# SuperbTUM/real-time-ReID-tracking

Hardware: AMD Instinct MI355X
Metric: crops/sec embedded + NxM distmat ms, ResNet18-SE 128x256 (higher is better)
Workload: dtype f16x3; 1 GPU; BASELINE configs[1]: ResNet18-SE embed 4096 distinct uint8 crops (128x256) per GPU + 4096x4096 L2 distmat; crops_per_gpu=4096, embed_dim=512, chunk=1024

## Files before the change

### include/reid_hip_debug.h

```cpp
#pragma once
#include "reid_hip.h"

#ifdef __cplusplus
extern "C" {
#endif

int reid_debug_set_switch(reid_ctx* ctx, const char* name, long long value);
int reid_debug_get_switch(reid_ctx* ctx, const char* name, long long* value);
int reid_debug_conv_f16(reid_ctx* ctx, int n, int h, int w, int cin, int cout, int r, int stride, int pad, int cfg, int iters,
                        float* ms_per_launch);
int reid_debug_conv_split(reid_ctx* ctx, int n, int h, int w, int c, int cout, int ablate, int iters, float* ms_per_launch);
int reid_debug_conv_f32(reid_ctx* ctx, int n, int h, int w, int cin, int cout, int r, int stride, int pad, int flags,
                        int variant, int iters, float* ms_per_launch);
int reid_debug_conv_c64(reid_ctx* ctx, int n, const float* x, const float* w_krsc, const float* scale, const float* shift,
                        const float* residual, int relu, float* out, float* stats);
int reid_debug_gemm_f16(reid_ctx* ctx, int m, int n, int k, int cfg, int iters, float* ms_per_launch,
                        unsigned long long* diag_host);
int reid_debug_linear(reid_ctx* ctx, int m, int n, int k, int mode, int iters, float* ms_per_launch);
int reid_debug_linear_rows(reid_ctx* ctx, const float* x, const float* w, const float* bias, const float* res, int m, int n, int k,
                           int mode, int flags, float* out);
int reid_debug_conv_layer(reid_ctx* ctx, const float* x, int n, int h, int w, int cin, const float* wgt, int cout, int r, int stride,
                          int pad, const float* scale, const float* shift, const float* residual, int relu, int relu_from, int pack_from,
                          int want_stats, const float* a_scale, const float* a_shift, int a_relu, float* out, uint16_t* packed,
                          float* stats, int* packed_written);
int reid_debug_norm_finish(reid_ctx* ctx, int form, int n, int hw, int c, int half, int tiles, const void* x, const float* stats,
                           const float* in_gamma, const float* in_beta, const float* bn_scale, const float* bn_shift, float* out,
                           uint16_t* out16, float* a_scale, float* a_shift);
int reid_debug_se_tail(reid_ctx* ctx, int form, int n, int hw, int c, int mid, int tiles, const float* stats, const float* w1,
                       const float* w2t, const void* y, const void* shortcut, float* out, uint16_t* out16, float* gate);
int reid_debug_sibling_tail(reid_ctx* ctx, int arch, int n, int h, int w, int c, const float* prm, const float* y, const float* shortcut,
                            float* out);
int reid_debug_gem_neck(reid_ctx* ctx, int f16, int n, int hw, int c, float p, const void* x, const float* scale, const float* shift,
                        float* gem_out, float* emb);
int reid_debug_stem(reid_ctx* ctx, int form, int is_u8, const void* x, int n, const float* w, const float* scale, const float* shift,
                    float* out, uint16_t* out16);
int reid_debug_resize_norm(reid_ctx* ctx, const uint8_t* packed, const long long* offsets, const int* hw, int n, int pitch, float* out);
int reid_debug_swin_crop_front(reid_ctx* ctx, const uint8_t* packed, const long long* offsets, const int* hw, int n, int pitch, int out_h,
                               int out_w, const float* mean_std6, const float* c1_w, const float* c1_b, float* out);
int reid_debug_swin_conv1(reid_ctx* ctx, const float* x, int n, int h, int w, const float* c1_w, const float* c1_b, float* out);
int reid_debug_maxpool(reid_ctx* ctx, int f16, const void* x, int n, int h, int w, int c, void* out);
int reid_debug_window_attn_cos(reid_ctx* ctx, int mode, const float* qkv, int n, int h, int w, int heads, int shifted, const float* bias,
                               const float* scale, float* out, uint16_t* out16);
int reid_debug_post_norm(reid_ctx* ctx, int side, const float* x, const float* y, int t, int c, const float* g, const float* b, int in_place,
                         float* out, uint16_t* out16);
int reid_debug_window_attn(reid_ctx* ctx, int form, const float* qkv, int n, int h, int w, int heads, int shifted, const float* pos169,
                           float* out, uint16_t* out16);
int reid_debug_layernorm(reid_ctx* ctx, int form, const float* x, int t, int c, const float* g, const float* b, float* out, uint16_t* out16);
int reid_debug_ln_linear(reid_ctx* ctx, const float* x, const float* ln_g, const float* ln_b, const float* w, const float* bias, int t, int c,
                         int n, float* out);
int reid_debug_swin_sfe(reid_ctx* ctx, const float* c1, int n, int h1, int w1, const float* in_g, const float* in_b, const float* bn_s,
                        const float* bn_t, const float* c2_w, const float* c2_b, const float* fc_w, const float* fc_b, float* ab, float* tok);
int reid_debug_swin_tail(reid_ctx* ctx, const float* x, int n, int ntok, const float* g, const float* b, float p, const float* bn_s,
                         const float* bn_t, float* gem, float* emb);
int reid_debug_swin_merge(reid_ctx* ctx, int stage, const float* x, int n, int h, int w, float* out);
int reid_debug_swin_fuse(reid_ctx* ctx, const float* sfe, const float* x1, const float* x2, const float* x3, const float* x4, int n, int h1,
                         int w1, void* a0, void* f3, void* f2, float* f1);
int reid_debug_two_linear_ablate(reid_ctx* ctx, int bits);
int reid_debug_two_linear(reid_ctx* ctx, const float* x, const float* w1, const float* b1, const float* w2, const float* b2,
                          const float* res, int m, int c, int hid, int act, int iters, float* out, float* ms, const float* ln_g,
                          const float* ln_b);
int reid_debug_select_exp(reid_ctx* ctx, int mode);
int reid_debug_knn_wide(reid_ctx* ctx, int enable, int force);
int reid_debug_conv_diag(reid_ctx* ctx, int enable, unsigned long long* out_host);
int reid_debug_mfma_shape(reid_ctx* ctx, int shape, int iters, int blocks, float* tflops);
int reid_debug_mfma_bare(reid_ctx* ctx, int shape, int zero, int iters, float* tflops);
int reid_debug_feed(reid_ctx* ctx, int mode, size_t footprint, int rowb, size_t stride, int iters, int inflight,
                    float* gbs_per_cu, float* tbs_chip);
int reid_debug_knn_merge(reid_ctx* ctx, const float* Dall, const int32_t* Iall, int world, int nq, int kk, int k, float* D,
                         int32_t* I);
int reid_debug_comm_loopback(reid_ctx** ctxs, int world);
int reid_debug_coissue(reid_ctx* ctx, int mode, int iters, int roles, double* cyc_mfma_wave, double* cyc_other_wave);

#ifdef __cplusplus
}
#endif
```

### real-time-reid-tracking_amd/_ffi.py

```python
import ctypes as C
import os

_HERE = os.path.dirname(os.path.abspath(__file__))
LIB_PATH = os.path.join(_HERE, "libreid_hip.so")
LIB_PATH = os.environ.get("REID_HIP_LIB", LIB_PATH)

METRIC_L2, METRIC_L2SQR, METRIC_COS_HALF, METRIC_COS, METRIC_DOT = range(5)
COMM_ID_BYTES = 128
K_CONV_GEMM, K_DIST_GEMM, K_ELEMENTWISE, K_SELECT = range(4)

_vp, _i, _sz = C.c_void_p, C.c_int, C.c_size_t
_SIGS = {
    "reid_last_error": (C.c_char_p, []),
    "reid_device_count": (_i, [C.POINTER(_i)]),
    "reid_ctx_create": (_i, [_i, C.POINTER(_vp)]),
    "reid_ctx_destroy": (_i, [_vp]),
    "reid_ctx_set_stream": (_i, [_vp, _vp]),
    "reid_ctx_set_null_stream": (_i, [_vp]),
    "reid_ctx_sync": (_i, [_vp]),
    "reid_device_sync": (_i, [_vp]),
    "reid_ctx_clear_fault": (_i, [_vp]),
    "reid_ctx_set_chunk": (_i, [_vp, _i]),
    "reid_ctx_set_precision": (_i, [_vp, _i]),
    "reid_ctx_precision_ok": (_i, [_vp, _i, _i]),
    "reid_ctx_fault_peek": (_i, [_vp, C.POINTER(_i)]),
    "reid_ctx_set_side_index": (_i, [_vp, _vp, _i]),
    "reid_malloc": (_i, [_vp, _sz, C.POINTER(_vp)]),
    "reid_free": (_i, [_vp, _vp]),
    "reid_memcpy_h2d": (_i, [_vp, _vp, _vp, _sz]),
    "reid_memcpy_d2h": (_i, [_vp, _vp, _vp, _sz]),
    "reid_timer_start": (_i, [_vp]),
    "reid_timer_stop": (_i, [_vp, C.POINTER(C.c_float)]),
    "reid_profile_enable": (_i, [_vp, _i]),
    "reid_profile_reset": (_i, [_vp]),
    "reid_profile_get": (_i, [_vp, _i, C.POINTER(C.c_double), C.POINTER(C.c_longlong), C.POINTER(C.c_double),
                              C.POINTER(C.c_double)]),
    "reid_seres18_load": (_i, [_vp, _vp, _sz, C.c_char_p]),
    "reid_seres18_dims": (_i, [_vp, C.POINTER(_i), C.POINTER(_i)]),
    "reid_embed_u8": (_i, [_vp, _vp, _i, _vp, _vp]),
    "reid_embed_u8_dev": (_i, [_vp, _vp, _i, _vp, _vp]),
    "reid_embed_ragged_u8": (_i, [_vp, _vp, _vp, _vp, _i, _vp, _vp]),
    "reid_embed_frame_u8": (_i, [_vp, _vp, _i, _i, _vp, _i, _vp, _vp]),
    "reid_embed_f32_nchw": (_i, [_vp, _vp, _i, _vp, _vp]),
    "reid_embed_f32_nchw_dev": (_i, [_vp, _vp, _i, _vp, _vp]),
    "reid_swin_load": (_i, [_vp, _vp, _sz, C.c_char_p]),
    "reid_swin_dims": (_i, [_vp, C.POINTER(_i), C.POINTER(_i)]),
    "reid_swin_embed_f32_nchw": (_i, [_vp, _vp, _i, _i, _i, _vp, _vp]),
    "reid_swin_embed_f32_nchw_dev": (_i, [_vp, _vp, _i, _i, _i, _vp, _vp]),
    "reid_swin_embed_ragged_u8": (_i, [_vp, _vp, _vp, _vp, _i, _i, _i, _vp, _vp, _vp]),
    "reid_swin_embed_frame_u8": (_i, [_vp, _vp, _i, _i, _vp, _i, _i, _i, _vp, _vp, _vp]),
    "reid_ctx_set_debug_keep": (_i, [_vp, _i]),
    "reid_debug_stage": (_i, [_vp, _i, _vp, _sz, C.POINTER(_sz)]),
    "reid_debug_swin_stage": (_i, [_vp, _i, _vp, _sz, C.POINTER(_sz)]),
    "reid_distmat": (_i, [_vp, _vp, _i, _vp, _i, _i, _i, _vp]),
    "reid_distmat_dev": (_i, [_vp, _vp, _i, _vp, _i, _i, _i, _vp]),
    "reid_argmin_rows": (_i, [_vp, _vp, _i, _vp, _i, _i, _i, _vp, _vp]),
    "reid_argmin_rows_dev": (_i, [_vp, _vp, _i, _vp, _i, _i, _i, _vp, _vp]),
    "reid_knn": (_i, [_vp, _vp, _i, _vp, _i, _i, _i, _vp, _vp]),
    "reid_knn_dev": (_i, [_vp, _vp, _i, _vp, _i, _i, _i, _vp, _vp]),
    "reid_descriptor_f32_nchw": (_i, [_vp, _vp, _i, _i, _vp]),
    "reid_descriptor_f32_nchw_dev": (_i, [_vp, _vp, _i, _i, _vp]),
    "reid_cam_debias": (_i, [_vp, _vp, _vp, _i, _i, C.c_float, _i]),
    "reid_cam_debias_dev": (_i, [_vp, _vp, _vp, _i, _i, C.c_float, _i]),
    "reid_smooth_tracklets": (_i, [_vp, _vp, _vp, _vp, _i, _i, C.c_float]),
    "reid_smooth_tracklets_dev": (_i, [_vp, _vp, _vp, _vp, _i, _i, C.c_float]),
    "reid_bank_create": (_i, [_vp, _i, _i, _i, C.POINTER(_vp)]),
    "reid_bank_destroy": (_i, [_vp]),
    "reid_bank_update": (_i, [_vp, _vp, _vp, _vp, _i]),
    "reid_bank_update_dev": (_i, [_vp, _vp, _vp, _vp, _i]),
    "reid_bank_clear": (_i, [_vp, _vp, _vp, _i]),
    "reid_bank_count": (_i, [_vp, _i, C.POINTER(_i)]),
    "reid_bank_cost": (_i, [_vp, _vp, _vp, _i, _vp, _i, _i, C.c_float, _vp]),
    "reid_bank_cost_dev": (_i, [_vp, _vp, _vp, _i, _vp, _i, _i, C.c_float, _vp]),
    "reid_host_alloc": (_i, [_vp, _sz, C.POINTER(_vp)]),
    "reid_host_free": (_i, [_vp, _vp]),
    "reid_frame_submit": (_i, [_vp, _i, _vp, _vp, _vp, _i]),
    "reid_frame_cost": (_i, [_vp, _i, _vp, _vp, _i, _i, C.c_float, _vp, _vp, _i]),
    "reid_frame_cost_groups": (_i, [_vp, _i, _i, _vp, _vp, _vp, _vp, _i, C.c_float, _vp, _vp, _i]),
    "reid_frame_match_stream": (_i, [_vp, _i]),
    "reid_frame_fetch": (_i, [_vp, _i, _vp, _vp, _vp]),
    "reid_frame_gather": (_i, [_vp, _i, _i]),
    "reid_frame_update": (_i, [_vp, _i, _vp, _vp, _vp, _i]),
    "reid_rerank_jaccard": (_i, [_vp, _vp, _i, _i, _i, _i, _vp, _vp]),
    "reid_rerank_jaccard_dev": (_i, [_vp, _vp, _i, _i, _i, _i, _vp, _vp]),
    "reid_diou": (_i, [_vp, _vp, _vp, _i, _vp]),
    "reid_diou_cost": (_i, [_vp, _vp, _i, _vp, _i, _vp]),
    "reid_rank_eval": (_i, [_vp, _vp, _vp, _vp, _i, _vp, _vp, _vp, _i, _i, _vp, _vp, _vp]),
    "reid_rank_eval_dev": (_i, [_vp, _vp, _vp, _vp, _i, _vp, _vp, _vp, _i, _i, _vp, _vp, _vp]),
    "reid_comm_unique_id": (_i, [_vp]),
    "reid_comm_init": (_i, [_vp, _i, _i, _vp]),
    "reid_comm_info": (_i, [_vp, C.POINTER(_i), C.POINTER(_i)]),
    "reid_comm_destroy": (_i, [_vp]),
    "reid_allgather_dev": (_i, [_vp, _vp, _vp, _sz]),
    "reid_allgather_rows_dev": (_i, [_vp, _vp, _i, _sz, _vp, _vp, C.POINTER(_i)]),
    "reid_allreduce_f64": (_i, [_vp, C.POINTER(C.c_double), _i, _i]),
    "reid_knn_gallery_sharded_dev": (_i, [_vp, _vp, _i, _vp, _i, _i, _i, _i, _vp, _vp]),
    "reid_conv2d_nhwc": (_i, [_vp, _vp, _i, _i, _i, _i, _vp, _i, _i, _i, _i, _i, _vp, _vp, _vp, _i, _vp]),
    "reid_gemm_nt": (_i, [_vp, _vp, _i, _vp, _i, _i, _vp, _vp]),
}
EXPORTS = tuple(sorted(_SIGS))

DEBUG_LIB_PATH = os.path.join(_HERE, "libreid_hip_debug.so")
DEBUG_EXPORTS = ("reid_debug_coissue", "reid_debug_comm_loopback", "reid_debug_conv_c64", "reid_debug_conv_layer", "reid_debug_conv_split", "reid_debug_conv_diag", "reid_debug_conv_f16", "reid_debug_conv_f32",
                 "reid_debug_feed", "reid_debug_gem_neck", "reid_debug_gemm_f16", "reid_debug_knn_merge", "reid_debug_knn_wide", "reid_debug_layernorm", "reid_debug_linear", "reid_debug_linear_rows", "reid_debug_ln_linear", "reid_debug_maxpool", "reid_debug_mfma_bare", "reid_debug_mfma_shape", "reid_debug_norm_finish", "reid_debug_post_norm", "reid_debug_resize_norm", "reid_debug_se_tail", "reid_debug_stem", "reid_debug_sibling_tail", "reid_debug_swin_conv1", "reid_debug_swin_crop_front", "reid_debug_swin_fuse", "reid_debug_swin_merge", "reid_debug_swin_sfe", "reid_debug_swin_tail", "reid_debug_select_exp", "reid_debug_set_switch", "reid_debug_get_switch", "reid_debug_two_linear", "reid_debug_two_linear_ablate", "reid_debug_window_attn", "reid_debug_window_attn_cos")

_lib = None
_dbg = None


class ReidHipError(RuntimeError):
    status = None


def lib():
    global _lib
    if _lib is None:
        if not os.path.exists(LIB_PATH):
            raise ReidHipError(
                "HIP extension missing: %s (build it with `python -c 'import __graft_entry__ as g; g.build()'` "
                "or `make -C real-time-reid-tracking_amd/csrc`); there is no CPU fallback" % LIB_PATH)
        l = C.CDLL(LIB_PATH, mode=C.RTLD_GLOBAL)
        for name, (res, args) in _SIGS.items():
            fn = getattr(l, name)
            fn.restype = res
            fn.argtypes = args
        _lib = l
    return _lib


def debug_lib():
    global _dbg
    if _dbg is None:
        lib()
        if not os.path.exists(DEBUG_LIB_PATH):
            raise ReidHipError("debug library missing: %s (make -C real-time-reid-tracking_amd/csrc)" % DEBUG_LIB_PATH)
        _dbg = C.CDLL(DEBUG_LIB_PATH)
    return _dbg


def check(status):
    if status != 0:
        msg = lib().reid_last_error()
        err = ReidHipError("libreid_hip status %d: %s" % (status, msg.decode() if msg else "?"))
        err.status = int(status)
        raise err
```

### real-time-reid-tracking_amd/csrc/api.hip

```cpp
#include "reid_internal.h"
#include "siblings_f16.h"
#include <dlfcn.h>
#include <mutex>
#include <stdarg.h>
#include <stdio.h>
#include <string.h>
#include <stdlib.h>
#include <sstream>

static thread_local char g_err[1024] = "";

void reid_set_error(const char* fmt, ...) {
    va_list ap;
    va_start(ap, fmt);
    vsnprintf(g_err, sizeof(g_err), fmt, ap);
    va_end(ap);
}

extern "C" const char* reid_last_error(void) { return g_err; }

extern "C" int reid_device_count(int* n) {
    ARG_CHECK(n);
    HIP_TRY(hipGetDeviceCount(n));
    return REID_OK;
// ... 636 lines not shown
    return launch_gemm_f32(ctx, amode, E_CONV, p, REID_K_CONV_GEMM, flops, bytes);
}

int conv_weights_fresh(reid_ctx* ctx, const float* d_w) {
    auto it = ctx->split_w.find(d_w);
    if (it != ctx->split_w.end()) {
        HIP_TRY(hipStreamSynchronize(ctx->stream));
        (void)hipFree(it->second);
        ctx->split_w.erase(it);
    }
    return REID_OK;
}

int conv_weights_splittable(reid_ctx* ctx, const float* h_w, size_t count, const char* who) {
    if (ctx->precision != 2) return REID_OK;
    for (size_t i = 0; i < count; ++i)
        if (!(fabsf(h_w[i]) * 2048.0f < 65504.0f)) {
            reid_set_error("%s: weight %zu (%g) is outside the range the fp32-class arithmetic (reid_ctx_set_precision 2) can split "
                           "(|w| 2^11 < 65504); use mode 0", who, i, (double)h_w[i]);
            return REID_ERR_ARG;
        }
    return REID_OK;
}

static int split_weights_of(reid_ctx* ctx, const float* wgt, int Cout, int taps, int Cin, const _Float16** out) {
    auto it = ctx->split_w.find(wgt);
    if (it == ctx->split_w.end()) {
        void* w16;
        HIP_TRY(hipMalloc(&w16, (size_t)Cout * taps * ctx->split_terms * Cin * 2));
        REID_TRY(launch_split_weights(ctx, wgt, Cout, taps, Cin, ctx->split_terms, (_Float16*)w16));
        it = ctx->split_w.emplace(wgt, w16).first;
    }
    *out = (const _Float16*)it->second;
    return REID_OK;
}

#ifdef REID_EXPERIMENTS
static int seres18_chain_layer4(reid_ctx* ctx, int n, const Se18Block& ka, const Se18Block& kb, const _Float16* in16, const float* sc,
                                float* y, float* out_a, float* out, float* stats) {
    const int H = 16, W = 8, hw = 128, C = 512, SK = 4, nnt = C / 128;
    const int nmt = (n * hw + 255) / 256;
    _Float16 *c1_16, *a16;
    float* skws;
    int* cnt;
    REID_TRY(ctx_ws(ctx, "split.c1", (size_t)n * hw * C * 2 * 2, (void**)&c1_16));
    REID_TRY(ctx_ws(ctx, "chain.a16", (size_t)n * hw * C * 2 * 2, (void**)&a16));
    const size_t part = (size_t)nmt * nnt * SK * 256 * 128;
    REID_TRY(ctx_ws(ctx, "chain.splitk", 4 * part * sizeof(float), (void**)&skws));
    const bool fresh = ctx->ws.find("chain.cnt") == ctx->ws.end();
    REID_TRY(ctx_ws(ctx, "chain.cnt", (4 * 1024 + 64 + 8 * 64) * sizeof(int), (void**)&cnt));
    if (fresh) HIP_TRY(hipMemsetAsync(cnt, 0, (4 * 1024 + 64 + 8 * 64) * sizeof(int), ctx->stream));
    ChainParams cp;
    memset(&cp, 0, sizeof(cp));
    cp.n_img = n;
    cp.flags = ctx->chain;
    cp.counters = cnt + 4 * 1024;
    cp.fault = ctx->fault;
    auto conv = [&](int idx, const _Float16* a, int cin, const float* wgt, const float* scale, const float* shift, const float* res, int relu,
                    float* stats_out, _Float16* pack) -> int {
        Gemm16Params& q = cp.conv[idx];
        q.H = H; q.W = W; q.Cin = 3 * cin; q.R = 3; q.S = 3; q.stride = 1; q.pad = 1; q.Ho = H; q.Wo = W;
        q.M = n * hw; q.N = C; q.K = 9 * 3 * cin; q.ldb = q.K;
        q.split_terms = 3;
        q.A = a;
        REID_TRY(split_weights_of(ctx, wgt, C, 9, cin, &q.B));
        q.C32 = y; q.ldc = C;
        q.col_scale = scale; q.col_shift = shift; q.res32 = res; q.relu = relu; q.relu_from = 0;
        q.stats = stats_out;
        q.acc_scale = 1.0f / 2048.0f;
        q.zero_page = ctx->se18.zero_page;
        q.pack16 = pack; q.pack_from = 0;
        q.split_k = SK; q.splitk_ws = skws + (size_t)idx * part; q.splitk_cnt = cnt + idx * 1024;
        q.fault = ctx->fault;
        return REID_OK;
    };
    REID_TRY(conv(0, in16, ka.cin, ka.conv1_w, ka.bn1_scale, ka.bn1_shift, nullptr, 1, nullptr, c1_16));
    REID_TRY(conv(1, c1_16, C, ka.conv2_w, ka.bn2_scale, ka.bn2_shift, nullptr, 0, stats, nullptr));
    REID_TRY(conv(2, a16, C, kb.conv1_w, kb.bn1_scale, kb.bn1_shift, nullptr, 1, nullptr, c1_16));
    REID_TRY(conv(3, c1_16, C, kb.conv2_w, kb.bn2_scale, kb.bn2_shift, out_a, 1, stats, nullptr));
    const int slices = 2;
    auto se = [&](int idx, const Se18Block& k, const float* shortcut, float* o, _Float16* pk) {
        ChainElem& e = cp.el[idx];
        e.x = y; e.stats = stats; e.sc = shortcut; e.g = k.se_w1; e.b = k.se_w2; e.out = o; e.packed = pk;
        e.c = C; e.half = 0; e.hw = hw; e.tiles = 1; e.mid = k.mid; e.slices = slices;
    };
    se(0, ka, sc, out_a, a16);
    se(1, kb, out_a, out, nullptr);
    const int conv_items = nmt * nnt * SK, se_items = n * slices;
    const int kinds[6] = {0, 0, 2, 0, 0, 2}, idxs[6] = {0, 1, 0, 2, 3, 1};
    const int targets[6] = {0, nnt * SK, nnt * SK, slices, nnt * SK, nnt * SK};
    int first = 0;
    for (int s = 0; s < 6; ++s) {
        ChainStage& st = cp.st[s];
        st.kind = kinds[s]; st.idx = idxs[s]; st.first = first; st.items = kinds[s] == 0 ? conv_items : se_items;
        st.dep = s - 1; st.target = targets[s]; st.sk = SK;
        first += st.items;
    }
    cp.n_stages = 6;
    cp.total_items = first;
    prof_begin(ctx, REID_K_CONV_GEMM, 2.0 * n * hw * C * 9.0 * (ka.cin + 3.0 * C), 0.0);
    const int st = launch_chain(ctx, cp, W);
    prof_end(ctx);
    return st;
}
#endif

struct Se18Bufs {
    float *stem, *pool, *t[4], *stats, *a_scale, *a_shift, *se, *gem;
    float* stage[11];
};

static int seres18_forward(reid_ctx* ctx, const void* x, bool is_u8, int n, float* d_emb, float* d_logits) {
    Se18Weights& w = ctx->se18;
    if (!w.loaded) {
        reid_set_error("reid_embed_*: call reid_seres18_load first");
        return REID_ERR_STATE;
    }
    Se18Bufs b;
    const size_t per = 131072;
    const bool keep = ctx->debug_keep != 0;
    REID_TRY(ctx_ws(ctx, "se18.stem", (size_t)n * 524288 * 4, (void**)&b.stem));
    REID_TRY(ctx_ws(ctx, "se18.pool", (size_t)n * per * 4, (void**)&b.pool));
    const int nt = keep ? 1 : 4;
    float* tbase = nullptr;
    REID_TRY(ctx_ws(ctx, "se18.t", (size_t)n * per * 4 * (keep ? 4 * 8 : 4), (void**)&tbase));
    REID_TRY(ctx_ws(ctx, "se18.stats", (size_t)n * 2048 * 4, (void**)&b.stats));
    REID_TRY(ctx_ws(ctx, "se18.ascale", (size_t)n * 512 * 4, (void**)&b.a_scale));
    REID_TRY(ctx_ws(ctx, "se18.ashift", (size_t)n * 512 * 4, (void**)&b.a_shift));
    REID_TRY(ctx_ws(ctx, "se18.se", (size_t)n * 512 * 4, (void**)&b.se));
    REID_TRY(ctx_ws(ctx, "se18.gem", (size_t)n * 512 * 4, (void**)&b.gem));
    (void)nt;

    const bool pool_fused = ctx->f32_conv == 1 && ctx->f32_stem_pool && ctx->debug_keep != 1;
    _Float16* cur16 = nullptr;
    const bool split_mode = ctx->precision == 2 && w.arch == 0 && ctx->f32_conv == 1;
    if (split_mode) REID_TRY(ctx_ws(ctx, "split.cur", (size_t)n * per * 2 * 2, (void**)&cur16));
    const bool stem_split = split_mode && pool_fused && ctx->stem_split;
    if (stem_split) {
        REID_TRY(launch_stem_split(ctx, x, is_u8, n, w.stem_w, w.stem_scale, w.stem_shift, b.pool, cur16));
    } else if (pool_fused) {
        REID_TRY(launch_stem_f32(ctx, x, is_u8, n, w.stem_w, w.stem_scale, w.stem_shift, b.pool, true));
    } else if (ctx->f32_conv == 1) {
        REID_TRY(launch_stem_f32(ctx, x, is_u8, n, w.stem_w, w.stem_scale, w.stem_shift, b.stem, false));
    } else {
        REID_TRY(conv_gemm(ctx, is_u8 ? A_STEM_U8 : A_STEM_F32, x, n, IMG_H, IMG_W, 3, w.stem_w, 64, 7, 7, 2, 3, 192, nullptr,
                           nullptr, 0, w.stem_scale, w.stem_shift, nullptr, 0, nullptr, b.stem));
    }
    if (!pool_fused) REID_TRY(launch_maxpool3s2(ctx, b.stem, n, 128, 64, 64, b.pool));
    b.stage[0] = b.stem;
    b.stage[1] = b.pool;

    const float* cur = b.pool;
    int H = 64, W = 32;
    if (split_mode && !stem_split) REID_TRY(launch_split_pack(ctx, b.pool, (long long)n * 64 * 32, 64, cur16));
    for (int i = 0; i < 8; ++i) {
        const Se18Block& k = w.blk[i];
#ifdef REID_EXPERIMENTS
        if (i == 6 && (ctx->chain & 1) && cur16 && !keep && n <= 64 && ctx->pack_epilogue && ctx->split_terms == 3) {
            float* fr[3];
            int nf = 0;
            for (int j = 0; j < 4 && nf < 3; ++j)
                if (tbase + (size_t)j * n * per != cur) fr[nf++] = tbase + (size_t)j * n * per;
            float *sc = fr[0], *y = fr[1], *out_a = fr[2], *out = const_cast<float*>(cur);
            REID_TRY(conv_gemm(ctx, A_IM2COL, cur, n, H, W, k.cin, k.ds_w, k.c, 1, 1, k.stride, 0, k.cin, nullptr, nullptr, 0, k.ds_scale, k.ds_shift,
                               nullptr, 0, nullptr, sc, 0, cur16));
            REID_TRY(seres18_chain_layer4(ctx, n, k, w.blk[7], cur16, sc, y, out_a, out, b.stats));
            b.stage[8] = out_a;
            b.stage[9] = out;
            cur = out;
            break;
        }
#endif
        float* tb[4];
        for (int j = 0; j < 4; ++j) tb[j] = tbase + ((size_t)(keep ? i * 4 : 0) + j) * n * per;
        float* free_[3];
        int nf = 0;
        for (int j = 0; j < 4 && nf < 3; ++j)
            if (tb[j] != cur) free_[nf++] = tb[j];
        float* c1 = free_[0];
        float* y = free_[1];
        float* sc = free_[2];
        const int Ho = (H + 2 - 3) / k.stride + 1, Wo = (W + 2 - 3) / k.stride + 1;
        const int hw = Ho * Wo, tiles = hw / 128;
        const int half = k.ibn ? k.c / 2 : 0;
        _Float16* c1_16 = nullptr;
        if (ctx->f32_conv == 1) {
            bool packed_c1 = false;
            if (cur16 && !keep && ctx->pack_epilogue) REID_TRY(ctx_ws(ctx, "split.c1", (size_t)n * hw * k.c * 2 * 2, (void**)&c1_16));
            if (k.ibn) {
                REID_TRY(conv_gemm(ctx, A_IM2COL, cur, n, H, W, k.cin, k.conv1_w, k.c, 3, 3, k.stride, 1, 9 * k.cin, nullptr, nullptr,
                                   0, w.ep + (size_t)i * 1024, w.ep + (size_t)i * 1024 + 512, nullptr, 1, b.stats, c1, half, cur16,
                                   c1_16, half, &packed_c1));
                if (cur16 && !keep) {
                    if (!c1_16) REID_TRY(ctx_ws(ctx, "split.c1", (size_t)n * hw * k.c * 2 * 2, (void**)&c1_16));
                    REID_TRY(launch_in_apply_pack(ctx, c1, b.stats, n, tiles, k.c, half, hw, k.in_gamma, k.in_beta, c1_16, packed_c1));
                } else {
                    REID_TRY(launch_in_apply(ctx, c1, b.stats, n, tiles, k.c, half, hw, k.in_gamma, k.in_beta));
                }
            } else {
                REID_TRY(conv_gemm(ctx, A_IM2COL, cur, n, H, W, k.cin, k.conv1_w, k.c, 3, 3, k.stride, 1, 9 * k.cin, nullptr, nullptr,
                                   0, k.bn1_scale, k.bn1_shift, nullptr, 1, nullptr, c1, 0, cur16, c1_16, 0, &packed_c1));
                if (!packed_c1) c1_16 = nullptr;
            }
            REID_TRY(conv_gemm(ctx, A_IM2COL, c1, n, Ho, Wo, k.c, k.conv2_w, k.c, 3, 3, 1, 1, 9 * k.c, nullptr, nullptr, 0,
                               k.bn2_scale, k.bn2_shift, k.ds ? nullptr : cur, k.ds ? 0 : 1, b.stats, y, 0, c1_16));
        } else {
        REID_TRY(conv_gemm(ctx, A_IM2COL, cur, n, H, W, k.cin, k.conv1_w, k.c, 3, 3, k.stride, 1, 9 * k.cin, nullptr, nullptr, 0,
                           nullptr, nullptr, nullptr, 0, b.stats, c1));
        REID_TRY(launch_norm_finalize(ctx, b.stats, n, tiles, k.c, half, hw, k.in_gamma, k.in_beta, k.bn1_scale, k.bn1_shift,
                                      b.a_scale, b.a_shift));
        REID_TRY(conv_gemm(ctx, A_IM2COL, c1, n, Ho, Wo, k.c, k.conv2_w, k.c, 3, 3, 1, 1, 9 * k.c, b.a_scale, b.a_shift, 1,
                           k.bn2_scale, k.bn2_shift, k.ds ? nullptr : cur, k.ds ? 0 : 1, b.stats, y));
        }
        const float* shortcut = cur;
        if (k.ds) {
            REID_TRY(conv_gemm(ctx, A_IM2COL, cur, n, H, W, k.cin, k.ds_w, k.c, 1, 1, k.stride, 0, k.cin, nullptr, nullptr, 0,
                               k.ds_scale, k.ds_shift, nullptr, 0, nullptr, sc, 0, cur16));
            shortcut = sc;
        }
        float* out = c1;
        if (w.arch == 1) {
            REID_TRY(launch_ta_tail(ctx, y, shortcut, n, Ho, Wo, k.c, k.ta, out));
        } else if (w.arch == 2) {
            REID_TRY(launch_ema_tail(ctx, y, shortcut, n, Ho, Wo, k.c, k.ema, out));
        } else if (ctx->f32_conv == 1) {
            bool fp32_read = true;
            if (cur16 && !keep && i < 7 && w.blk[i + 1].ds && ctx->pack_epilogue) {
                const Se18Block& nx = w.blk[i + 1];
                fp32_read = !(conv_split_path(ctx, n, Ho, Wo, nx.cin, nx.c, 3, 3, nx.stride, 1) &&
                              conv_split_path(ctx, n, Ho, Wo, nx.cin, nx.c, 1, 1, nx.stride, 0));
            }
            REID_TRY(launch_se_tail(ctx, b.stats, n, tiles, k.c, k.mid, hw, k.se_w1, k.se_w2, y, shortcut, fp32_read ? out : nullptr,
                                    i < 7 ? cur16 : nullptr));
        } else {
            REID_TRY(launch_se_finalize(ctx, b.stats, n, tiles, k.c, k.mid, hw, k.se_w1, k.se_w2, b.se));
            REID_TRY(launch_se_combine(ctx, y, shortcut, b.se, n, hw, k.c, out));
        }
        b.stage[2 + i] = out;
        cur = out;
        H = Ho;
        W = Wo;
    }
    REID_TRY(launch_gem_neck(ctx, cur, n, H * W, 512, w.gem_p, w.neck_scale, w.neck_shift, b.gem, d_emb));
    {
        const int32_t* d_cam;
        REID_TRY(ctx_take_side(ctx, n, w.num_cams, "reid_embed (camera bias)", &d_cam));
        if (d_cam) REID_TRY(launch_add_indexed_rows(ctx, d_emb, n, 1, 512, w.cam_bias, d_cam, w.cam_factor));
    }
    b.stage[10] = b.gem;
    if (d_logits) {
        if (!w.cls_w) {
            reid_set_error("logits requested but the weight blob has no classifier (cls.w)");
            return REID_ERR_STATE;
        }
        GemmParams p;
        memset(&p, 0, sizeof(p));
        p.A = d_emb; p.lda = 512;
        p.B = w.cls_w; p.ldb = 512;
        p.M = n; p.N = w.num_class; p.K = 512;
        p.C = d_logits; p.ldc = w.num_class;
        REID_TRY(launch_gemm_f32(ctx, A_DENSE, E_BIAS, p, REID_K_CONV_GEMM, 2.0 * n * w.num_class * 512,
                                 ((double)n * 512 + (double)w.num_class * 512 + (double)n * w.num_class) * 4.0));
    }
    ctx->last_n = n;
    ctx->last_f16 = false;
    for (int s = 0; s < 11; ++s) ctx->stage_ptr[s] = b.stage[s];
    return REID_OK;
}

struct SiblingsF16Api {
    decltype(&siblings_f16_ta_workspace_bytes) ta_bytes = nullptr;
    decltype(&siblings_f16_ta_tail) ta = nullptr;
    decltype(&siblings_f16_ema_tail) ema = nullptr;
};
static int siblings_f16_api(const SiblingsF16Api** out) {
    static std::mutex m;
    static SiblingsF16Api api;
    std::lock_guard<std::mutex> lk(m);
    if (!api.ta) {
        Dl_info info;
        std::string path = "libreid_hip_siblings_f16.so";
        if (dladdr((const void*)&siblings_f16_api, &info) && info.dli_fname) {
            const std::string self = info.dli_fname;
            const size_t slash = self.rfind('/');
            if (slash != std::string::npos) path = self.substr(0, slash + 1) + path;
        }
        void* h = dlopen(path.c_str(), RTLD_NOW | RTLD_LOCAL);
        if (!h) {
            reid_set_error("CARes18-IBN / EMARes18-IBN in the fp16-storage mode need %s beside libreid_hip.so: %s", path.c_str(), dlerror());
            return REID_ERR_STATE;
        }
        auto b = (decltype(api.ta_bytes))dlsym(h, "siblings_f16_ta_workspace_bytes");
        auto t = (decltype(api.ta))dlsym(h, "siblings_f16_ta_tail");
        auto e = (decltype(api.ema))dlsym(h, "siblings_f16_ema_tail");
        if (!b || !t || !e) {
            dlclose(h);
            reid_set_error("%s lacks siblings_f16_ta_workspace_bytes / siblings_f16_ta_tail / siblings_f16_ema_tail", path.c_str());
            return REID_ERR_STATE;
        }
        api.ta_bytes = b;
        api.ema = e;
        api.ta = t;
    }
    *out = &api;
    return REID_OK;
}

static int launch_sibling_tail_f16(reid_ctx* ctx, const SiblingsF16Api* api, int arch, const _Float16* y, const _Float16* sc, int n, int H,
                                   int W, int C, const float* prm, _Float16* out) {
    ARG_CHECK(api && y && sc && prm && out && out != y && out != sc);
    void* ws = nullptr;
    if (arch == 1) {
        const size_t bytes = api->ta_bytes(n, H, W, C);
        ARG_CHECK(bytes > 0);
        REID_TRY(ctx_ws(ctx, "ta16.ws", bytes, &ws));
    }
    prof_begin(ctx, REID_K_ELEMENTWISE, 0, (double)n * H * W * C * 2.0 * 4.0);
    const hipError_t e = arch == 1 ? api->ta(ctx->stream, y, sc, n, H, W, C, prm, ws, out) : api->ema(ctx->stream, y, sc, n, H, W, C, prm, out);
    prof_end(ctx);
    HIP_TRY(e);
    return REID_OK;
}

int conv_gemm16(reid_ctx* ctx, int amode, const _Float16* x, int n, int H, int W, int Cin, const _Float16* wgt, int Cout,
                       int R, int S, int stride, int pad, int K, const float* col_scale, const float* col_shift,
                       const _Float16* residual, int relu, float* stats, _Float16* out, int Hp, int Wp) {
    Gemm16Params p;
    memset(&p, 0, sizeof(p));
    p.A = x;
    p.H = H; p.W = W; p.Cin = Cin; p.R = R; p.S = S; p.stride = stride; p.pad = pad; p.Hp = Hp; p.Wp = Wp;
    p.Ho = (H + 2 * pad - R) / stride + 1;
    p.Wo = (W + 2 * pad - S) / stride + 1;
    p.B = wgt; p.ldb = amode == A16_STEM ? 256 : K;
    p.M = n * p.Ho * p.Wo; p.N = Cout; p.K = K;
    p.C = out; p.ldc = Cout;
    p.col_scale = col_scale; p.col_shift = col_shift; p.residual = residual; p.relu = relu; p.stats = stats;
    p.zero_page = ctx->se18.zero_page;
    p.diag = ctx->conv_diag;
    const double ktrue = (double)R * S * (amode == A16_STEM ? 3 : Cin);
    const double flops = 2.0 * p.M * Cout * ktrue;
    const double bytes = ((double)n * H * W * (amode == A16_STEM ? 4 : Cin) + (double)p.M * Cout + (double)Cout * ktrue +
                          (residual ? (double)p.M * Cout : 0.0)) * 2.0;
    if (amode == A16_IM2COL && ctx->f16_halo && conv3x3_f16_supported(p)) {
        if (ctx->f16_halo == 2 || Cout >= 128) return launch_conv3x3_f16(ctx, p, REID_K_CONV_GEMM, flops, bytes);
    }
    return launch_gemm_f16(ctx, amode, p, REID_K_CONV_GEMM, flops, bytes);
}

static const int PAD_H = 262, PAD_W = 136;

static int seres18_forward_f16(reid_ctx* ctx, const void* x, bool is_u8, int n, float* d_emb, float* d_logits) {
    Se18Weights& w = ctx->se18;
    if (!w.loaded) {
        reid_set_error("reid_embed_*: call reid_seres18_load first");
        return REID_ERR_STATE;
    }
    typedef _Float16 f16;
    const size_t per = 131072;
    const bool keep = ctx->debug_keep != 0;
    const bool sibling = w.arch != 0;
    const SiblingsF16Api* sib = nullptr;
    if (sibling) REID_TRY(siblings_f16_api(&sib));
    f16 *pad_in, *stem, *pool, *tbase;
    float *stats, *a_scale, *a_shift, *se, *gem;
    REID_TRY(ctx_ws(ctx, "se18h.pad", (size_t)n * PAD_H * PAD_W * 4 * 2, (void**)&pad_in));
    REID_TRY(ctx_ws(ctx, "se18h.stem", (size_t)n * 524288 * 2, (void**)&stem));
    REID_TRY(ctx_ws(ctx, "se18h.pool", (size_t)n * per * 2, (void**)&pool));
    REID_TRY(ctx_ws(ctx, "se18h.t", (size_t)n * per * 2 * (keep ? 4 * 8 : 4), (void**)&tbase));
    REID_TRY(ctx_ws(ctx, "se18.stats", (size_t)n * 2048 * 4, (void**)&stats));
    REID_TRY(ctx_ws(ctx, "se18.ascale", (size_t)n * 512 * 4, (void**)&a_scale));
    REID_TRY(ctx_ws(ctx, "se18.ashift", (size_t)n * 512 * 4, (void**)&a_shift));
    REID_TRY(ctx_ws(ctx, "se18.se", (size_t)n * 512 * 4, (void**)&se));
    REID_TRY(ctx_ws(ctx, "se18.gem", (size_t)n * 512 * 4, (void**)&gem));

    const bool per_image_ok = n >= 128 || ctx->debug_keep == 2;
    const bool fused = ctx->f16_stem_fused && ctx->debug_keep != 1 && per_image_ok;
    if (is_u8 && fused && ctx->f16_stem_fused == 2) {
        REID_TRY(launch_stem_pool_f16(ctx, nullptr, (const uint8_t*)x, n, w.stem_w16s, w.stem_shift, pool));
    } else if (fused) {
        if (is_u8) REID_TRY(launch_prep_u8_pad_f16(ctx, (const uint8_t*)x, n, IMG_H, IMG_W, PAD_H, PAD_W, pad_in));
        else REID_TRY(launch_prep_f32_pad_f16(ctx, (const float*)x, n, IMG_H, IMG_W, PAD_H, PAD_W, pad_in));
        REID_TRY(launch_stem_pool_f16(ctx, pad_in, nullptr, n, w.stem_w16s, w.stem_shift, pool));
    } else {
        if (is_u8) REID_TRY(launch_prep_u8_pad_f16(ctx, (const uint8_t*)x, n, IMG_H, IMG_W, PAD_H, PAD_W, pad_in));
        else REID_TRY(launch_prep_f32_pad_f16(ctx, (const float*)x, n, IMG_H, IMG_W, PAD_H, PAD_W, pad_in));
        REID_TRY(conv_gemm16(ctx, A16_STEM, pad_in, n, IMG_H, IMG_W, 4, w.stem_w16, 64, 7, 7, 2, 3, 224, w.stem_scale,
                             w.stem_shift, nullptr, 0, nullptr, stem, PAD_H, PAD_W));
        REID_TRY(launch_maxpool3s2_f16(ctx, stem, n, 128, 64, 64, pool));
    }
    float* stage[11];
    stage[0] = (float*)stem;
    stage[1] = (float*)pool;

    const f16* cur = pool;
    int H = 64, W = 32;
    for (int i = 0; i < 8; ++i) {
// ... 735 lines not shown
```

### real-time-reid-tracking_amd/csrc/debug.hip

```cpp
#include "reid_internal.h"
#include <string.h>
#include <stdlib.h>
#include <vector>

namespace {
struct Switch { const char* name; int reid_ctx::* field; };
const Switch kSwitches[] = {
    {"f16_cfg", &reid_ctx::f16_cfg}, {"f16_lin_256", &reid_ctx::f16_lin_256}, {"f16_split_k", &reid_ctx::f16_split_k},
    {"bank_fast", &reid_ctx::bank_fast}, {"side_copy", &reid_ctx::side_copy}, {"f32_stem_pool", &reid_ctx::f32_stem_pool},
    {"stem_split", &reid_ctx::stem_split}, {"split_pair", &reid_ctx::split_pair}, {"split_lean_epi", &reid_ctx::split_lean_epi},
    {"knn_wide", &reid_ctx::knn_wide}, {"f16_loader_prio", &reid_ctx::f16_loader_prio}, {"f16_frag_ahead", &reid_ctx::f16_frag_ahead},
    {"pack_epilogue", &reid_ctx::pack_epilogue}, {"f16_wide_splitk", &reid_ctx::f16_wide_splitk}, {"f32_split_k", &reid_ctx::f32_split_k},
    {"swin_fold", &reid_ctx::swin_fold}, {"swin_stop", &reid_ctx::swin_stop}, {"select_two_pass", &reid_ctx::select_two_pass},
    {"split_terms", &reid_ctx::split_terms}, {"f32_conv", &reid_ctx::f32_conv}, {"swin_attn_mfma", &reid_ctx::swin_attn_mfma},
    {"swin_attn_split", &reid_ctx::swin_attn_split}, {"swin_two_linear", &reid_ctx::swin_two_linear},
    {"f16_loader_waves", &reid_ctx::f16_loader_waves}, {"f16_halo", &reid_ctx::f16_halo}, {"f16_stem_fused", &reid_ctx::f16_stem_fused},
    {"f16_se_tail", &reid_ctx::f16_se_tail}, {"f16_c64", &reid_ctx::f16_c64}, {"swin_chunk_cap", &reid_ctx::swin_chunk_cap},
    {"split_x3", &reid_ctx::split_x3}, {"x3_ablate", &reid_ctx::x3_ablate}, {"x3_unroll", &reid_ctx::x3_unroll}, {"x3_narrow", &reid_ctx::x3_narrow}, {"conv_x3s", &reid_ctx::conv_x3s}, {"x3s_sk_cap", &reid_ctx::x3s_sk_cap}, {"x3_l4_narrow_nmt", &reid_ctx::x3_l4_narrow_nmt}, {"split_x3_small", &reid_ctx::split_x3_small}, {"split_x3_min_blocks", &reid_ctx::split_x3_min_blocks}, {"f32_dist_bk16", &reid_ctx::f32_dist_bk16}, {"lin_x3", &reid_ctx::lin_x3},
    {"host_pipeline", &reid_ctx::host_pipeline}, {"x3_sk_cap", &reid_ctx::x3_sk_cap}, {"chain", &reid_ctx::chain}, {"split_gemm_min_tiles", &reid_ctx::split_gemm_min_tiles},
    {"rerank_hbm_acc", &reid_ctx::rerank_hbm_acc},
};
}

extern "C" int reid_debug_set_switch(reid_ctx* ctx, const char* name, long long value) {
    ARG_CHECK(ctx && name);
    CTX_GUARD(ctx);
    HIP_TRY(hipStreamSynchronize(ctx->stream));
    if (!strcmp(name, "knn_wide_min")) {
        ctx->knn_wide_min = value;
        return REID_OK;
    }
    for (const Switch& s : kSwitches)
        if (!strcmp(name, s.name)) {
            if (!strcmp(name, "split_terms") && value != 3 && value != 4) break;
            ctx->*(s.field) = (int)value;
            return REID_OK;
        }
    reid_set_error("reid_debug_set_switch: no switch '%s' (or a value it does not take)", name);
    return REID_ERR_ARG;
}

extern "C" int reid_debug_get_switch(reid_ctx* ctx, const char* name, long long* value) {
    ARG_CHECK(ctx && name && value);
    if (!strcmp(name, "knn_wide_min")) {
        *value = ctx->knn_wide_min;
        return REID_OK;
    }
    for (const Switch& s : kSwitches)
        if (!strcmp(name, s.name)) {
            *value = ctx->*(s.field);
            return REID_OK;
        }
    reid_set_error("reid_debug_get_switch: no switch '%s'", name);
    return REID_ERR_ARG;
}

extern "C" int reid_debug_conv_f16(reid_ctx* ctx, int n, int h, int w, int cin, int cout, int r, int stride, int pad, int cfg,
                                   int iters, float* ms_per_launch) {
    ARG_CHECK(ctx && ms_per_launch && ctx->se18.loaded);
    CTX_GUARD(ctx);
    typedef _Float16 f16;
    const int ho = (h + 2 * pad - r) / stride + 1, wo = (w + 2 * pad - r) / stride + 1;
    const size_t nin = (size_t)n * h * w * cin, nw = (size_t)cout * r * r * cin, nout = (size_t)n * ho * wo * cout;
    f16 *x, *wt, *out;
    REID_TRY(ctx_ws(ctx, "dbg.x", nin * 2, (void**)&x));
    REID_TRY(ctx_ws(ctx, "dbg.w", nw * 2, (void**)&wt));
    REID_TRY(ctx_ws(ctx, "dbg.out", nout * 2, (void**)&out));
    const size_t src_n = ctx->se18.n_floats;
    for (size_t o = 0; o < nin; o += src_n) REID_TRY(launch_f32_to_f16(ctx, ctx->se18.blob, nin - o < src_n ? nin - o : src_n, x + o));
    for (size_t o = 0; o < nw; o += src_n) REID_TRY(launch_f32_to_f16(ctx, ctx->se18.blob, nw - o < src_n ? nw - o : src_n, wt + o));
    if (getenv("REID_DEBUG_ZERO")) {
        HIP_TRY(hipMemsetAsync(x, 0, nin * 2, ctx->stream));
        HIP_TRY(hipMemsetAsync(wt, 0, nw * 2, ctx->stream));
    }
    const int c0 = ctx->f16_cfg;
    const int h0 = ctx->f16_halo;
    ctx->f16_halo = cfg >= 2000000 ? 2 : 0;
    const int l0 = ctx->f16_loader_waves;
    if (cfg >= 2000000) ctx->f16_loader_waves = cfg & 1;
    ctx->f16_cfg = cfg >= 2000000 ? 0 : cfg;
    int st = REID_OK;
    for (int i = 0; i < 2 && st == REID_OK; ++i)
        st = conv_gemm16(ctx, A16_IM2COL, x, n, h, w, cin, wt, cout, r, r, stride, pad, r * r * cin, nullptr, nullptr, nullptr, 0, nullptr, out);
    if (st == REID_OK) st = reid_timer_start(ctx);
    for (int i = 0; i < iters && st == REID_OK; ++i)
        st = conv_gemm16(ctx, A16_IM2COL, x, n, h, w, cin, wt, cout, r, r, stride, pad, r * r * cin, nullptr, nullptr, nullptr, 0, nullptr, out);
    float ms = 0.f;
    if (st == REID_OK) st = reid_timer_stop(ctx, &ms);
    ctx->f16_cfg = c0;
    ctx->f16_halo = h0;
    ctx->f16_loader_waves = l0;
    *ms_per_launch = ms / (iters > 0 ? iters : 1);
    return st;
}


extern "C" int reid_debug_conv_split(reid_ctx* ctx, int n, int h, int w, int c, int cout, int ablate, int iters, float* ms_per_launch) {
    ARG_CHECK(ctx && ms_per_launch && ctx->se18.loaded && c % 64 == 0 && cout % 64 == 0);
    CTX_GUARD(ctx);
    typedef _Float16 f16;
    const size_t nin = (size_t)n * h * w * 2 * c, nw = (size_t)cout * 9 * 3 * c, nout = (size_t)n * h * w * cout;
    f16 *x, *wt;
    float *out, *sc;
    REID_TRY(ctx_ws(ctx, "dbgs.x", nin * 2, (void**)&x));
    REID_TRY(ctx_ws(ctx, "dbgs.w", nw * 2, (void**)&wt));
    REID_TRY(ctx_ws(ctx, "dbgs.out", nout * 4, (void**)&out));
    REID_TRY(ctx_ws(ctx, "dbgs.sc", (size_t)cout * 2 * 4, (void**)&sc));
    const size_t src_n = ctx->se18.n_floats;
    for (size_t o = 0; o < nin; o += src_n) REID_TRY(launch_f32_to_f16(ctx, ctx->se18.blob, nin - o < src_n ? nin - o : src_n, x + o));
    for (size_t o = 0; o < nw; o += src_n) REID_TRY(launch_f32_to_f16(ctx, ctx->se18.blob, nw - o < src_n ? nw - o : src_n, wt + o));
    HIP_TRY(hipMemcpyAsync(sc, ctx->se18.blob, (size_t)cout * 2 * 4, hipMemcpyDeviceToDevice, ctx->stream));
    if (ablate & 128) {
        HIP_TRY(hipMemsetAsync(x, 0, nin * 2, ctx->stream));
        HIP_TRY(hipMemsetAsync(wt, 0, nw * 2, ctx->stream));
    }
    Gemm16Params q;
    memset(&q, 0, sizeof(q));
    q.split_terms = 3;
    q.H = h; q.W = w; q.Cin = 3 * c; q.R = 3; q.S = 3; q.stride = 1; q.pad = 1; q.Ho = h; q.Wo = w;
    q.M = n * h * w; q.N = cout; q.K = 27 * c; q.ldb = q.K;
    q.A = x; q.B = wt; q.C32 = out; q.ldc = cout;
    q.col_scale = sc; q.col_shift = sc + cout; q.relu = 1;
    q.acc_scale = 1.0f / 2048.0f;
    q.zero_page = ctx->se18.zero_page;
    q.ablate = ablate & 127;
    q.diag = ctx->conv_diag;
    int st = REID_OK;
    for (int i = 0; i < 2 && st == REID_OK; ++i) st = launch_conv3x3_split(ctx, q, REID_K_CONV_GEMM, 0, 0);
    if (st == REID_OK) st = reid_timer_start(ctx);
    for (int i = 0; i < iters && st == REID_OK; ++i) st = launch_conv3x3_split(ctx, q, REID_K_CONV_GEMM, 0, 0);
    float ms = 0.f;
    if (st == REID_OK) st = reid_timer_stop(ctx, &ms);
    *ms_per_launch = ms / (iters > 0 ? iters : 1);
    return st;
}

extern "C" int reid_debug_conv_c64(reid_ctx* ctx, int n, const float* x, const float* w_krsc, const float* scale,
                                   const float* shift, const float* residual, int relu, float* out, float* stats) {
    ARG_CHECK(ctx && x && w_krsc && out && n >= 1);
    CTX_GUARD(ctx);
    typedef _Float16 f16;
    const size_t nact = (size_t)n * 64 * 32 * 64, nw = 64 * 576;
    float *xf, *wf, *rf = nullptr, *sc = nullptr, *sh = nullptr, *st = nullptr, *of;
    f16 *xh, *wh, *rh = nullptr, *oh, *zp;
    REID_TRY(ctx_ws(ctx, "dbg64.xf", nact * 4, (void**)&xf));
    REID_TRY(ctx_ws(ctx, "dbg64.wf", nw * 4, (void**)&wf));
    REID_TRY(ctx_ws(ctx, "dbg64.xh", nact * 2, (void**)&xh));
    REID_TRY(ctx_ws(ctx, "dbg64.wh", nw * 2, (void**)&wh));
    REID_TRY(ctx_ws(ctx, "dbg64.oh", nact * 2, (void**)&oh));
    REID_TRY(ctx_ws(ctx, "dbg64.of", nact * 4, (void**)&of));
    REID_TRY(ctx_ws(ctx, "dbg64.zp", 256, (void**)&zp));
    REID_TRY(ctx_ws(ctx, "dbg64.sc", 64 * 4, (void**)&sc));
    REID_TRY(ctx_ws(ctx, "dbg64.sh", 64 * 4, (void**)&sh));
    REID_TRY(ctx_ws(ctx, "dbg64.st", (size_t)n * 128 * 4, (void**)&st));
    HIP_TRY(hipMemsetAsync(zp, 0, 256, ctx->stream));
    HIP_TRY(hipMemcpyAsync(xf, x, nact * 4, hipMemcpyHostToDevice, ctx->stream));
    HIP_TRY(hipMemcpyAsync(wf, w_krsc, nw * 4, hipMemcpyHostToDevice, ctx->stream));
    std::vector<float> ones(64, 1.f);
    HIP_TRY(hipMemcpyAsync(sc, scale ? scale : ones.data(), 64 * 4, hipMemcpyHostToDevice, ctx->stream));
    if (shift) HIP_TRY(hipMemcpyAsync(sh, shift, 64 * 4, hipMemcpyHostToDevice, ctx->stream));
    REID_TRY(launch_f32_to_f16(ctx, xf, nact, xh));
    REID_TRY(launch_scale_rows_f16(ctx, wf, sc, 64, 576, wh));
    if (residual) {
        REID_TRY(ctx_ws(ctx, "dbg64.rf", nact * 4, (void**)&rf));
        REID_TRY(ctx_ws(ctx, "dbg64.rh", nact * 2, (void**)&rh));
        HIP_TRY(hipMemcpyAsync(rf, residual, nact * 4, hipMemcpyHostToDevice, ctx->stream));
        REID_TRY(launch_f32_to_f16(ctx, rf, nact, rh));
    }
    HIP_TRY(hipStreamSynchronize(ctx->stream));
    REID_TRY(launch_conv3x3_c64_f16(ctx, xh, n, wh, shift ? sh : nullptr, rh, relu, stats ? st : nullptr, oh, zp));
    std::vector<f16> tmp(nact);
    HIP_TRY(hipMemcpyAsync(tmp.data(), oh, nact * 2, hipMemcpyDeviceToHost, ctx->stream));
    if (stats) HIP_TRY(hipMemcpyAsync(stats, st, (size_t)n * 128 * 4, hipMemcpyDeviceToHost, ctx->stream));
// ... 309 lines not shown

namespace {
template <class T>
int dbg_upload(reid_ctx* ctx, const char* name, const T* host, size_t count, T** dev) {
    *dev = nullptr;
    if (!host) return REID_OK;
    REID_TRY(ctx_ws(ctx, name, count * sizeof(T), (void**)dev));
    HIP_TRY(hipMemcpyAsync(*dev, host, count * sizeof(T), hipMemcpyHostToDevice, ctx->stream));
    return REID_OK;
}
template <class T>
int dbg_output(reid_ctx* ctx, const char* name, size_t count, T** dev) {
    REID_TRY(ctx_ws(ctx, name, count * sizeof(T), (void**)dev));
    HIP_TRY(hipMemsetAsync(*dev, 0xff, count * sizeof(T), ctx->stream));
    return REID_OK;
}
template <class T>
int dbg_download(reid_ctx* ctx, T* host, const T* dev, size_t count) {
    if (host) HIP_TRY(hipMemcpyAsync(host, dev, count * sizeof(T), hipMemcpyDeviceToHost, ctx->stream));
    return REID_OK;
}
}

extern "C" int reid_debug_norm_finish(reid_ctx* ctx, int form, int n, int hw, int c, int half, int tiles, const void* x, const float* stats,
                                      const float* in_gamma, const float* in_beta, const float* bn_scale, const float* bn_shift, float* out,
                                      uint16_t* out16, float* a_scale, float* a_shift) {
    ARG_CHECK(ctx && form >= 0 && form <= 5 && n >= 1 && hw >= 1 && c >= 4 && half >= 4 && half <= c && tiles >= 1 && stats && in_gamma &&
              in_beta);
    ARG_CHECK((form == 0 || x) && (form != 1 || out) && (form < 2 || form > 5 || out16) && (form != 0 || (a_scale && a_shift)));
    ARG_CHECK((form != 0 && form < 4) || half == c || (bn_scale && bn_shift));
    CTX_ENTER(ctx);
    const size_t nx = (size_t)n * hw * c, nab = (size_t)n * c, cb = (size_t)(c - half);
    float *dst, *dg, *db, *dbs = nullptr, *dbh = nullptr, *dx = nullptr, *da = nullptr, *dbb = nullptr;
    _Float16* dh = nullptr;
    REID_TRY(dbg_upload(ctx, "dbgt.stats", stats, (size_t)n * tiles * c * 2, &dst));
    REID_TRY(dbg_upload(ctx, "dbgt.gamma", in_gamma, (size_t)half, &dg));
    REID_TRY(dbg_upload(ctx, "dbgt.beta", in_beta, (size_t)half, &db));
    if (cb) {
        REID_TRY(dbg_upload(ctx, "dbgt.bns", bn_scale, cb, &dbs));
        REID_TRY(dbg_upload(ctx, "dbgt.bnh", bn_shift, cb, &dbh));
    }
    if (form == 0 || form == 5) {
        REID_TRY(dbg_output(ctx, "dbgt.a", nab, &da));
        REID_TRY(dbg_output(ctx, "dbgt.b", nab, &dbb));
    }
    if (form >= 1 && form <= 3) REID_TRY(dbg_upload(ctx, "dbgt.x", (const float*)x, nx, &dx));
    if (form >= 4) REID_TRY(dbg_upload(ctx, "dbgt.x16", (const _Float16*)x, nx, &dh));
    if (form == 2 || form == 3) REID_TRY(dbg_output(ctx, "dbgt.pk", nx * 2, &dh));
    switch (form) {
    case 0: REID_TRY(launch_norm_finalize(ctx, dst, n, tiles, c, half, hw, dg, db, dbs, dbh, da, dbb)); break;
    case 1: REID_TRY(launch_in_apply(ctx, dx, dst, n, tiles, c, half, hw, dg, db)); break;
    case 2:
    case 3: REID_TRY(launch_in_apply_pack(ctx, dx, dst, n, tiles, c, half, hw, dg, db, dh, form == 3)); break;
    case 4: REID_TRY(launch_norm_apply_f16(ctx, dh, dst, n, tiles, c, half, hw, dg, db, dbs, dbh)); break;
    case 5:
        REID_TRY(launch_norm_finalize(ctx, dst, n, tiles, c, half, hw, dg, db, dbs, dbh, da, dbb));
        REID_TRY(launch_affine_relu_f16(ctx, dh, da, dbb, n, hw, c));
        break;
    }
    if (dx) REID_TRY(dbg_download(ctx, out, dx, nx));
    if (dh) REID_TRY(dbg_download(ctx, (_Float16*)out16, dh, form == 2 || form == 3 ? nx * 2 : nx));
    if (da) {
        REID_TRY(dbg_download(ctx, a_scale, da, nab));
        REID_TRY(dbg_download(ctx, a_shift, dbb, nab));
    }
    HIP_TRY(hipStreamSynchronize(ctx->stream));
    return ctx_fault_status(ctx);
}

extern "C" int reid_debug_se_tail(reid_ctx* ctx, int form, int n, int hw, int c, int mid, int tiles, const float* stats, const float* w1,
                                  const float* w2t, const void* y, const void* shortcut, float* out, uint16_t* out16, float* gate) {
    ARG_CHECK(ctx && form >= 0 && form <= 11 && n >= 1 && hw >= 1 && c >= 4 && mid >= 1 && tiles >= 1 && stats && w1 && w2t && y && shortcut);
    const bool f16 = form >= 10, tail = form >= 1 && form <= 9;
    const bool want_out = !f16 && (!tail || ((form - 1) % 3 != 1)), want_pk = tail && (form - 1) % 3 != 0;
    ARG_CHECK((!want_out || out) && ((!want_pk && !f16) || out16) && ((form != 0 && form != 11) || gate));
    CTX_ENTER(ctx);
    const size_t ny = (size_t)n * hw * c;
    float *dst, *dw1, *dw2, *dy = nullptr, *dsc = nullptr, *dout = nullptr, *dgate = nullptr;
    _Float16 *dy16 = nullptr, *dsc16 = nullptr, *dh = nullptr;
    REID_TRY(dbg_upload(ctx, "dbgt.stats", stats, (size_t)n * tiles * c * 2, &dst));
    REID_TRY(dbg_upload(ctx, "dbgt.w1", w1, (size_t)mid * c, &dw1));
    REID_TRY(dbg_upload(ctx, "dbgt.w2", w2t, (size_t)mid * c, &dw2));
    if (f16) {
        REID_TRY(dbg_upload(ctx, "dbgt.x16", (const _Float16*)y, ny, &dy16));
        REID_TRY(dbg_upload(ctx, "dbgt.sc16", (const _Float16*)shortcut, ny, &dsc16));
        REID_TRY(dbg_output(ctx, "dbgt.pk", ny, &dh));
    } else {
        REID_TRY(dbg_upload(ctx, "dbgt.x", (const float*)y, ny, &dy));
        REID_TRY(dbg_upload(ctx, "dbgt.sc", (const float*)shortcut, ny, &dsc));
        if (want_out) REID_TRY(dbg_output(ctx, "dbgt.out", ny, &dout));
        if (want_pk) REID_TRY(dbg_output(ctx, "dbgt.pk", ny * 2, &dh));
    }
    if (form == 0 || form == 11) REID_TRY(dbg_output(ctx, "dbgt.a", (size_t)n * c, &dgate));
    if (form == 0) {
        REID_TRY(launch_se_finalize(ctx, dst, n, tiles, c, mid, hw, dw1, dw2, dgate));
        REID_TRY(launch_se_combine(ctx, dy, dsc, dgate, n, hw, c, dout));
    } else if (tail) {
        REID_TRY(launch_se_tail_form(ctx, (form - 1) / 3 - 1, dst, n, tiles, c, mid, hw, dw1, dw2, dy, dsc, dout, dh));
    } else if (form == 10) {
        REID_TRY(launch_se_tail_f16(ctx, dst, n, tiles, c, mid, hw, dw1, dw2, dy16, dsc16, dh));
    } else {
        REID_TRY(launch_se_finalize(ctx, dst, n, tiles, c, mid, hw, dw1, dw2, dgate));
        REID_TRY(launch_se_combine_f16(ctx, dy16, dsc16, dgate, n, hw, c, dh));
    }
    if (dout) REID_TRY(dbg_download(ctx, out, dout, ny));
    if (dh) REID_TRY(dbg_download(ctx, (_Float16*)out16, dh, f16 ? ny : ny * 2));
    if (dgate) REID_TRY(dbg_download(ctx, gate, dgate, (size_t)n * c));
    HIP_TRY(hipStreamSynchronize(ctx->stream));
    return ctx_fault_status(ctx);
}

extern "C" int reid_debug_sibling_tail(reid_ctx* ctx, int arch, int n, int h, int w, int c, const float* prm, const float* y,
                                       const float* shortcut, float* out) {
    ARG_CHECK(ctx && (arch == 1 || arch == 2) && n >= 1 && h >= 1 && w >= 1 && c >= 32 && c % 32 == 0 && prm && y && shortcut && out);
    CTX_ENTER(ctx);
    const size_t ny = (size_t)n * h * w * c, cg = (size_t)c / 32;
    float *dp, *dy, *dsc, *dout;
    REID_TRY(dbg_upload(ctx, "dbgt.w1", prm, arch == 1 ? (size_t)300 : cg * cg * 10 + 4 * cg, &dp));
    REID_TRY(dbg_upload(ctx, "dbgt.x", y, ny, &dy));
    REID_TRY(dbg_upload(ctx, "dbgt.sc", shortcut, ny, &dsc));
    REID_TRY(dbg_output(ctx, "dbgt.out", ny, &dout));
    if (arch == 1) REID_TRY(launch_ta_tail(ctx, dy, dsc, n, h, w, c, dp, dout));
    else REID_TRY(launch_ema_tail(ctx, dy, dsc, n, h, w, c, dp, dout));
    REID_TRY(dbg_download(ctx, out, dout, ny));
    HIP_TRY(hipStreamSynchronize(ctx->stream));
    return ctx_fault_status(ctx);
}

extern "C" int reid_debug_gem_neck(reid_ctx* ctx, int f16, int n, int hw, int c, float p, const void* x, const float* scale,
                                   const float* shift, float* gem_out, float* emb) {
    ARG_CHECK(ctx && n >= 1 && hw >= 1 && c >= 64 && x && scale && shift && emb);
    CTX_ENTER(ctx);
    const size_t nx = (size_t)n * hw * c, ne = (size_t)n * c;
    float *dx = nullptr, *dp, *dsc, *dsh, *dg = nullptr, *de;
    _Float16* dh = nullptr;
    REID_TRY(dbg_upload(ctx, "dbgt.p", &p, 1, &dp));
    REID_TRY(dbg_upload(ctx, "dbgt.bns", scale, (size_t)c, &dsc));
    REID_TRY(dbg_upload(ctx, "dbgt.bnh", shift, (size_t)c, &dsh));
    if (gem_out) REID_TRY(dbg_output(ctx, "dbgt.a", ne, &dg));
    REID_TRY(dbg_output(ctx, "dbgt.b", ne, &de));
    if (f16) {
        REID_TRY(dbg_upload(ctx, "dbgt.x16", (const _Float16*)x, nx, &dh));
        REID_TRY(launch_gem_neck_f16(ctx, dh, n, hw, c, dp, dsc, dsh, dg, de));
    } else {
        REID_TRY(dbg_upload(ctx, "dbgt.x", (const float*)x, nx, &dx));
        REID_TRY(launch_gem_neck(ctx, dx, n, hw, c, dp, dsc, dsh, dg, de));
    }
    if (dg) REID_TRY(dbg_download(ctx, gem_out, dg, ne));
    REID_TRY(dbg_download(ctx, emb, de, ne));
    HIP_TRY(hipStreamSynchronize(ctx->stream));
    return ctx_fault_status(ctx);
}

extern "C" int reid_debug_two_linear_ablate(reid_ctx* ctx, int bits) {
    ARG_CHECK(ctx && bits >= 0 && bits < 4);
    ctx->two_linear_ablate = bits;
    return REID_OK;
}

extern "C" int reid_debug_two_linear(reid_ctx* ctx, const float* x, const float* w1, const float* b1, const float* w2, const float* b2,
                                     const float* res, int m, int c, int hid, int act, int iters, float* out, float* ms, const float* ln_g,
                                     const float* ln_b) {
    ARG_CHECK(ctx && x && w1 && b1 && w2 && b2 && res && out && m > 0 && iters >= 1);
    CTX_GUARD(ctx);
    ARG_CHECK(two_linear_supported(ctx, m, c, hid));
    typedef _Float16 f16;
    float *x32, *dw1, *dw2, *db1, *db2, *r32, *o32;
    f16* a16;
    REID_TRY(ctx_ws(ctx, "dbg2.x", (size_t)m * c * 4, (void**)&x32));
    REID_TRY(ctx_ws(ctx, "dbg2.w1", (size_t)hid * c * 4, (void**)&dw1));
    REID_TRY(ctx_ws(ctx, "dbg2.w2", (size_t)hid * c * 4, (void**)&dw2));
    REID_TRY(ctx_ws(ctx, "dbg2.b1", (size_t)hid * 4, (void**)&db1));
    REID_TRY(ctx_ws(ctx, "dbg2.b2", (size_t)c * 4, (void**)&db2));
    REID_TRY(ctx_ws(ctx, "dbg2.res", (size_t)m * c * 4, (void**)&r32));
    REID_TRY(ctx_ws(ctx, "dbg2.out", (size_t)m * c * 4, (void**)&o32));
    REID_TRY(ctx_ws(ctx, "dbg2.a16", (size_t)m * 2 * c * 2, (void**)&a16));
    float *dg = nullptr, *dbt = nullptr;
    if (ln_g && ln_b) {
        REID_TRY(ctx_ws(ctx, "dbg2.lng", (size_t)c * 4, (void**)&dg));
        REID_TRY(ctx_ws(ctx, "dbg2.lnb", (size_t)c * 4, (void**)&dbt));
        HIP_TRY(hipMemcpyAsync(dg, ln_g, (size_t)c * 4, hipMemcpyHostToDevice, ctx->stream));
        HIP_TRY(hipMemcpyAsync(dbt, ln_b, (size_t)c * 4, hipMemcpyHostToDevice, ctx->stream));
    }
    const _Float16* ain = dg ? nullptr : a16;
    HIP_TRY(hipMemcpyAsync(x32, x, (size_t)m * c * 4, hipMemcpyHostToDevice, ctx->stream));
    HIP_TRY(hipMemcpyAsync(dw1, w1, (size_t)hid * c * 4, hipMemcpyHostToDevice, ctx->stream));
    HIP_TRY(hipMemcpyAsync(dw2, w2, (size_t)hid * c * 4, hipMemcpyHostToDevice, ctx->stream));
    HIP_TRY(hipMemcpyAsync(db1, b1, (size_t)hid * 4, hipMemcpyHostToDevice, ctx->stream));
    HIP_TRY(hipMemcpyAsync(db2, b2, (size_t)c * 4, hipMemcpyHostToDevice, ctx->stream));
    HIP_TRY(hipMemcpyAsync(r32, res, (size_t)m * c * 4, hipMemcpyHostToDevice, ctx->stream));
    REID_TRY(launch_split_pack(ctx, x32, m, c, a16));
    for (const void* key : {(const void*)((const char*)dw1 + 1), (const void*)((const char*)dw2 + 1)}) {
        auto it = ctx->split_w.find(key);
        if (it != ctx->split_w.end()) {
            HIP_TRY(hipStreamSynchronize(ctx->stream));
            (void)hipFree(it->second);
            ctx->split_w.erase(it);
        }
    }
    REID_TRY(launch_two_linear(ctx, ain, m, c, hid, dw1, db1, dw2, db2, act, r32, o32, x32, dg, dbt));
    if (iters > 1) {
        hipEvent_t e0, e1;
        HIP_TRY(hipEventCreate(&e0));
        HIP_TRY(hipEventCreate(&e1));
        HIP_TRY(hipEventRecord(e0, ctx->stream));
        for (int i = 0; i < iters; ++i) REID_TRY(launch_two_linear(ctx, ain, m, c, hid, dw1, db1, dw2, db2, act, r32, o32, x32, dg, dbt));
        HIP_TRY(hipEventRecord(e1, ctx->stream));
        HIP_TRY(hipEventSynchronize(e1));
        float t = 0.f;
        HIP_TRY(hipEventElapsedTime(&t, e0, e1));
        if (ms) *ms = t / iters;
        (void)hipEventDestroy(e0);
        (void)hipEventDestroy(e1);
    }
    HIP_TRY(hipMemcpyAsync(out, o32, (size_t)m * c * 4, hipMemcpyDeviceToHost, ctx->stream));
    HIP_TRY(hipStreamSynchronize(ctx->stream));
    return REID_OK;
}

#include <condition_variable>
#include <chrono>
#include <mutex>

namespace {
struct LoopComm : reid_comm_loop {
    int world, attached;
    std::mutex mu;
    std::condition_variable cv;
    int arrived = 0;
    long gen = 0;
    std::vector<const void*> send;
    std::vector<double> red;
    explicit LoopComm(int w) : world(w), attached(w), send(w, nullptr), red((size_t)w * 64, 0.0) {}

    bool barrier() {
        std::unique_lock<std::mutex> lk(mu);
        const long g = gen;
        if (++arrived == world) {
            arrived = 0;
            ++gen;
            cv.notify_all();
            return true;
        }
        return cv.wait_for(lk, std::chrono::seconds(60), [&] { return gen != g; });
    }
    int allgather(int rank, const void* d_send, void* d_recv, size_t bytes, hipStream_t st) override {
        HIP_TRY(hipStreamSynchronize(st));
        send[rank] = d_send;
        if (!barrier()) { reid_set_error("loop-back all-gather: rank %d waited 60 s for the others", rank); return REID_ERR_STATE; }
        for (int r = 0; r < world; ++r)
            HIP_TRY(hipMemcpyAsync((char*)d_recv + (size_t)r * bytes, send[r], bytes, hipMemcpyDeviceToDevice, st));
        HIP_TRY(hipStreamSynchronize(st));
        if (!barrier()) { reid_set_error("loop-back all-gather: rank %d waited 60 s for the others", rank); return REID_ERR_STATE; }
        return REID_OK;
    }
    int allreduce(int rank, double* inout, int count, int op) override {
        for (int i = 0; i < count; ++i) red[(size_t)rank * 64 + i] = inout[i];
        if (!barrier()) { reid_set_error("loop-back all-reduce: rank %d waited 60 s for the others", rank); return REID_ERR_STATE; }
        for (int i = 0; i < count; ++i) {
            double v = red[i];
            for (int r = 1; r < world; ++r) v = op == 0 ? v + red[(size_t)r * 64 + i] : (red[(size_t)r * 64 + i] > v ? red[(size_t)r * 64 + i] : v);
            inout[i] = v;
        }
        if (!barrier()) { reid_set_error("loop-back all-reduce: rank %d waited 60 s for the others", rank); return REID_ERR_STATE; }
        return REID_OK;
    }
    void detach(int) override {
        bool last;
        {
            std::lock_guard<std::mutex> lk(mu);
            last = --attached == 0;
        }
        if (last) delete this;
    }
};
}

extern "C" int reid_debug_comm_loopback(reid_ctx** ctxs, int world) {
    ARG_CHECK(ctxs && world >= 1 && world <= 64);
    for (int r = 0; r < world; ++r) {
        ARG_CHECK(ctxs[r] && ctxs[r]->device == ctxs[0]->device);
        for (int q = 0; q < r; ++q) ARG_CHECK(ctxs[q] != ctxs[r]);
        if (ctxs[r]->comm) {
            reid_set_error("reid_debug_comm_loopback: context %d already has a communicator", r);
            return REID_ERR_STATE;
        }
    }
    LoopComm* lc = new LoopComm(world);
    for (int r = 0; r < world; ++r) {
        reid_comm* c = new reid_comm();
        c->rank = r;
        c->world = world;
        c->loop = lc;
        ctxs[r]->comm = c;
    }
    return REID_OK;
}

extern "C" int reid_debug_window_attn_cos(reid_ctx* ctx, int mode, const float* qkv, int n, int h, int w, int heads, int shifted,
                                          const float* bias, const float* scale, float* out, uint16_t* out16) {
    ARG_CHECK(ctx && mode >= 0 && mode <= 2 && qkv && bias && scale && n >= 1 && heads >= 1 && heads <= 64 && h >= 7 && w >= 7 && h % 7 == 0 &&
              w % 7 == 0);
    ARG_CHECK(mode == 0 ? out != nullptr : out16 != nullptr);
    CTX_ENTER(ctx);
    const int C = heads * 32;
    const size_t T = (size_t)n * h * w;
// ... 403 lines not shown
```

### real-time-reid-tracking_amd/csrc/elementwise.hip

```cpp
#include "reid_internal.h"
#include <math.h>

typedef float f32x4 __attribute__((ext_vector_type(4)));

namespace {

__device__ __forceinline__ float wave_sum(float v) {
#pragma unroll
    for (int o = 32; o > 0; o >>= 1) v += __shfl_xor(v, o);
    return v;
}
__device__ __forceinline__ double wave_sum_d(double v) {
#pragma unroll
    for (int o = 32; o > 0; o >>= 1) v += __shfl_xor(v, o);
    return v;
}

__global__ void nchw_to_nhwc3_kernel(const float* __restrict__ x, long long npix, int hw, float* __restrict__ out) {
    for (long long i = blockIdx.x * (long long)blockDim.x + threadIdx.x; i < npix; i += (long long)gridDim.x * blockDim.x) {
        const long long img = i / hw;
        const int p = (int)(i - img * hw);
        const float* src = x + img * 3 * hw + p;
        float* dst = out + i * 3;
        dst[0] = src[0];
        dst[1] = src[hw];
        dst[2] = src[2 * hw];
    }
}

__device__ __forceinline__ void lin_tap(int d, int dst, int src, int& s, float& f) {
#pragma clang fp contract(off)
    const double scale = (double)src / (double)dst;
    float fx = (float)(((double)d + 0.5) * scale - 0.5);
    int sx = (int)floorf(fx);
    fx = fx - (float)sx;
    if (sx < 0) { sx = 0; fx = 0.f; }
    if (sx >= src - 1) { sx = src - 1; fx = 0.f; }
    s = sx;
    f = fx;
}
__global__ void resize_norm_kernel(const uint8_t* __restrict__ packed, const long long* __restrict__ offsets,
                                   const int* __restrict__ hw, int n, int H, int W, int pitch, float* __restrict__ out) {
#pragma clang fp contract(off)
    const long long total = (long long)n * H * W;
    for (long long i = blockIdx.x * (long long)blockDim.x + threadIdx.x; i < total; i += (long long)gridDim.x * blockDim.x) {
        const int img = (int)(i / (H * W));
        const int rem = (int)(i - (long long)img * H * W);
        const int dy = rem / W, dx = rem - dy * W;
        const int h = hw[2 * img], w = hw[2 * img + 1];
        const uint8_t* src = packed + offsets[img];
        const long long ps = pitch ? pitch : w;
        int sx, sy;
        float fx, fy;
        lin_tap(dx, W, w, sx, fx);
        lin_tap(dy, H, h, sy, fy);
        const int sx1 = min(sx + 1, w - 1), sy1 = min(sy + 1, h - 1);
        const float gx = 1.0f - fx, gy = 1.0f - fy;
#pragma unroll
        for (int c = 0; c < 3; ++c) {
            const float p00 = (float)src[(sy * ps + sx) * 3 + c] / 255.0f;
            const float p01 = (float)src[(sy * ps + sx1) * 3 + c] / 255.0f;
            const float p10 = (float)src[(sy1 * ps + sx) * 3 + c] / 255.0f;
            const float p11 = (float)src[(sy1 * ps + sx1) * 3 + c] / 255.0f;
            const float r0 = p00 * gx + p01 * fx;
            const float r1 = p10 * gx + p11 * fx;
            const float v = r0 * gy + r1 * fy;
            out[i * 3 + c] = (v - 0.5f) / 0.5f;
        }
    }
}

__global__ void maxpool3s2_kernel(const float* __restrict__ x, int n, int h, int w, int c, int ho, int wo,
                                  float* __restrict__ out) {
    const int c4n = c >> 2;
    const long long total = (long long)n * ho * wo * c4n;
    for (long long i = blockIdx.x * (long long)blockDim.x + threadIdx.x; i < total; i += (long long)gridDim.x * blockDim.x) {
        const int cc = (int)(i % c4n);
        long long t = i / c4n;
        const int ox = (int)(t % wo);
        t /= wo;
        const int oy = (int)(t % ho);
        const int img = (int)(t / ho);
        f32x4 m = {-INFINITY, -INFINITY, -INFINITY, -INFINITY};
#pragma unroll
        for (int dy = 0; dy < 3; ++dy) {
            const int iy = oy * 2 - 1 + dy;
            if ((unsigned)iy >= (unsigned)h) continue;
#pragma unroll
            for (int dx = 0; dx < 3; ++dx) {
                const int ix = ox * 2 - 1 + dx;
                if ((unsigned)ix >= (unsigned)w) continue;
                const f32x4 v = *(const f32x4*)(x + (((long long)img * h + iy) * w + ix) * c + cc * 4);
                m.x = fmaxf(m.x, v.x); m.y = fmaxf(m.y, v.y); m.z = fmaxf(m.z, v.z); m.w = fmaxf(m.w, v.w);
            }
        }
        *(f32x4*)(out + (((long long)img * ho + oy) * wo + ox) * c + cc * 4) = m;
    }
}

__global__ void norm_finalize_kernel(const float* __restrict__ stats, int tiles, int c, int half, int hw,
                                     const float* __restrict__ in_gamma, const float* __restrict__ in_beta,
                                     const float* __restrict__ bn_scale, const float* __restrict__ bn_shift,
                                     float* __restrict__ a_scale, float* __restrict__ a_shift) {
    const int img = blockIdx.x;
    for (int ch = threadIdx.x; ch < c; ch += blockDim.x) {
        float a, b;
        if (ch < half) {
            double s1 = 0.0, s2 = 0.0;
            for (int t = 0; t < tiles; ++t) {
                const float* st = stats + (((long long)img * tiles + t) * c + ch) * 2;
                s1 += (double)st[0];
                s2 += (double)st[1];
            }
            const double mean = s1 / hw;
            double var = s2 / hw - mean * mean;
            if (var < 0.0) var = 0.0;
            const double inv = 1.0 / sqrt(var + 1e-5);
            a = (float)(inv * (double)in_gamma[ch]);
            b = (float)((double)in_beta[ch] - mean * inv * (double)in_gamma[ch]);
        } else {
            a = bn_scale[ch - half];
            b = bn_shift[ch - half];
        }
        a_scale[(long long)img * c + ch] = a;
        a_shift[(long long)img * c + ch] = b;
    }
}

__global__ __launch_bounds__(256) void in_apply_kernel(float* __restrict__ x, const float* __restrict__ stats, int tiles, int c,
                                                       int half, int hw, int rows, const float* __restrict__ in_gamma,
                                                       const float* __restrict__ in_beta) {
    __shared__ float sa[256], sb[256];
    const int img = blockIdx.y, tid = threadIdx.x;
    for (int ch = tid; ch < half; ch += 256) {
        double s1 = 0.0, s2 = 0.0;
        for (int t = 0; t < tiles; ++t) {
            const float* st = stats + (((long long)img * tiles + t) * c + ch) * 2;
            s1 += (double)st[0];
            s2 += (double)st[1];
        }
        const double mean = s1 / hw;
        double var = s2 / hw - mean * mean;
        if (var < 0.0) var = 0.0;
        const double inv = 1.0 / sqrt(var + 1e-5);
        sa[ch] = (float)(inv * (double)in_gamma[ch]);
        sb[ch] = (float)((double)in_beta[ch] - mean * inv * (double)in_gamma[ch]);
    }
    __syncthreads();
    const int q = half >> 2;
    float* base = x + ((long long)img * hw + (long long)blockIdx.x * rows) * c;
    for (int i = tid; i < rows * q; i += 256) {
        const int row = i / q, cc = i - row * q;
        f32x4* ptr = (f32x4*)(base + (long long)row * c + cc * 4);
        f32x4 v = *ptr;
        const f32x4 a = *(const f32x4*)&sa[cc * 4], b = *(const f32x4*)&sb[cc * 4];
        v = v * a + b;
        v.x = fmaxf(v.x, 0.f); v.y = fmaxf(v.y, 0.f); v.z = fmaxf(v.z, 0.f); v.w = fmaxf(v.w, 0.f);
        *ptr = v;
    }
}

__global__ __launch_bounds__(256) void in_apply_pack_kernel(const float* __restrict__ x, const float* __restrict__ stats, int tiles, int c,
                                                            int half, int hw, int rows, const float* __restrict__ in_gamma,
                                                            const float* __restrict__ in_beta, _Float16* __restrict__ packed, int in_only,
                                                            int* __restrict__ fault) {
    __shared__ float sa[512], sb[512];
    const int img = blockIdx.y, tid = threadIdx.x;
    for (int ch = tid; ch < c; ch += 256) {
        if (ch >= half) {
            sa[ch] = 1.f;
            sb[ch] = 0.f;
            continue;
        }
        double s1 = 0.0, s2 = 0.0;
        for (int t = 0; t < tiles; ++t) {
            const float* st = stats + (((long long)img * tiles + t) * c + ch) * 2;
            s1 += (double)st[0];
            s2 += (double)st[1];
        }
        const double mean = s1 / hw;
        double var = s2 / hw - mean * mean;
        if (var < 0.0) var = 0.0;
        const double inv = 1.0 / sqrt(var + 1e-5);
        sa[ch] = (float)(inv * (double)in_gamma[ch]);
        sb[ch] = (float)((double)in_beta[ch] - mean * inv * (double)in_gamma[ch]);
    }
    __syncthreads();
    const int q = (in_only ? half : c) >> 2;
    const long long pix0 = (long long)img * hw + (long long)blockIdx.x * rows;
    typedef _Float16 h4 __attribute__((ext_vector_type(4)));
    unsigned vm = 0u;
    for (int i = tid; i < rows * q; i += 256) {
        const int row = i / q, cc = i - row * q;
        f32x4 v = *(const f32x4*)(x + (pix0 + row) * c + cc * 4);
        if (cc * 4 < half) {
            const f32x4 a = *(const f32x4*)&sa[cc * 4], b = *(const f32x4*)&sb[cc * 4];
            v = v * a + b;
            vm = range_acc(range_acc(range_acc(range_acc(vm, v.x), v.y), v.z), v.w);
            v.x = fmaxf(v.x, 0.f); v.y = fmaxf(v.y, 0.f); v.z = fmaxf(v.z, 0.f); v.w = fmaxf(v.w, 0.f);
        } else {
            vm = range_acc(range_acc(range_acc(range_acc(vm, v.x), v.y), v.z), v.w);
        }
        const h4 hi = {(_Float16)v.x, (_Float16)v.y, (_Float16)v.z, (_Float16)v.w};
        const h4 lo = {(_Float16)((v.x - (float)hi.x) * 2048.0f), (_Float16)((v.y - (float)hi.y) * 2048.0f),
                       (_Float16)((v.z - (float)hi.z) * 2048.0f), (_Float16)((v.w - (float)hi.w) * 2048.0f)};
        *(h4*)(packed + (pix0 + row) * 2 * c + cc * 4) = hi;
        *(h4*)(packed + (pix0 + row) * 2 * c + c + cc * 4) = lo;
    }
    range_raise(fault, vm);
}

__global__ __launch_bounds__(256) void se_finalize_kernel(const float* __restrict__ stats, int tiles, int c, int mid,
                                                          int hw, const float* __restrict__ w1,
                                                          const float* __restrict__ w2, float* __restrict__ s) {
    __shared__ float pooled[512];
    __shared__ float hid[64];
    const int img = blockIdx.x, tid = threadIdx.x, lane = tid & 63, wave = tid >> 6;
    for (int ch = tid; ch < c; ch += 256) {
        double acc = 0.0;
        for (int t = 0; t < tiles; ++t) acc += (double)stats[(((long long)img * tiles + t) * c + ch) * 2];
        pooled[ch] = (float)(acc / hw);
    }
    __syncthreads();
    for (int m = wave; m < mid; m += 4) {
        float acc = 0.f;
        for (int ch = lane; ch < c; ch += 64) acc += w1[m * c + ch] * pooled[ch];
        acc = wave_sum(acc);
        if (lane == 0) hid[m] = fmaxf(acc, 0.f);
    }
    __syncthreads();
    for (int ch = tid; ch < c; ch += 256) {
        float acc = 0.f;
        for (int m = 0; m < mid; ++m) acc += w2[m * c + ch] * hid[m];
        s[(long long)img * c + ch] = 1.0f / (1.0f + expf(-acc));
    }
}

__global__ void se_combine_kernel(const float* __restrict__ y, const float* __restrict__ sc, const float* __restrict__ s,
                                  long long total4, int hw, int c, float* __restrict__ out) {
    const int c4n = c >> 2;
    for (long long i = blockIdx.x * (long long)blockDim.x + threadIdx.x; i < total4; i += (long long)gridDim.x * blockDim.x) {
        const int cc = (int)(i % c4n);
        const long long pix = i / c4n;
        const long long img = pix / hw;
        const f32x4 yy = *(const f32x4*)(y + i * 4);
        const f32x4 rr = *(const f32x4*)(sc + i * 4);
        const f32x4 ss = *(const f32x4*)(s + img * c + cc * 4);
        f32x4 o = ss * yy + rr;
        o.x = fmaxf(o.x, 0.f); o.y = fmaxf(o.y, 0.f); o.z = fmaxf(o.z, 0.f); o.w = fmaxf(o.w, 0.f);
        *(f32x4*)(out + i * 4) = o;
    }
}

template <bool SMALL>
__global__ __launch_bounds__(256) void se_tail_kernel(const float* __restrict__ stats, int tiles, int c, int mid, int hw,
                                                      const float* __restrict__ w1, const float* __restrict__ w2,
                                                      const float* __restrict__ y, const float* __restrict__ sc, int rows,
                                                      float* __restrict__ out, _Float16* __restrict__ packed, int* __restrict__ fault) {
    __shared__ __attribute__((aligned(16))) float pooled[512];
    __shared__ float hid[64];
    __shared__ __attribute__((aligned(16))) float gate[512];
    const int img = blockIdx.y, tid = threadIdx.x, lane = tid & 63, wave = tid >> 6;
    constexpr int MJ = SMALL ? 8 : 16, MW2 = 32;
    f32x4 w1v[SMALL ? 8 : 1][2];
    float w2v[SMALL ? 2 : 1][SMALL ? MW2 : 1];
    if constexpr (SMALL) {
        const int c4v = c >> 2;
#pragma unroll
        for (int j = 0; j < MJ; ++j)
#pragma unroll
            for (int k = 0; k < 2; ++k) {
                const int m = wave + 4 * j, c4 = lane + 64 * k;
                if (m < mid && c4 < c4v) w1v[j][k] = *(const f32x4*)(w1 + (long long)m * c + c4 * 4);
            }
#pragma unroll
        for (int q = 0; q < 2; ++q)
#pragma unroll
            for (int m = 0; m < MW2; ++m) {
                const int ch = tid + 256 * q;
                if (ch < c && m < mid) w2v[q][m] = w2[m * c + ch];
            }
    }
    for (int ch = tid; ch < c; ch += 256) {
        double acc = 0.0;
        for (int t = 0; t < tiles; ++t) acc += (double)stats[(((long long)img * tiles + t) * c + ch) * 2];
        pooled[ch] = (float)(acc / hw);
    }
    __syncthreads();
    {
        const int c4v = c >> 2;
        float acc[16];
#pragma unroll
        for (int j = 0; j < 16; ++j) {
            acc[j] = 0.f;
            if (SMALL && j >= MJ) continue;
            const int m = wave + 4 * j;
#pragma unroll
            for (int k = 0; k < 2; ++k) {
                const int c4 = lane + 64 * k;
                if (m < mid && c4 < c4v) {
                    f32x4 wv;
                    if constexpr (SMALL) wv = w1v[j < MJ ? j : 0][k];
                    else wv = *(const f32x4*)(w1 + (long long)m * c + c4 * 4);
                    const f32x4 pv = *(const f32x4*)(pooled + c4 * 4);
                    acc[j] += wv.x * pv.x + wv.y * pv.y + wv.z * pv.z + wv.w * pv.w;
                }
            }
        }
#pragma unroll
        for (int j = 0; j < 16; ++j) {
            if (wave + 4 * j < mid) {
                const float v = wave_sum(acc[j]);
                if (lane == 0) hid[wave + 4 * j] = fmaxf(v, 0.f);
            }
        }
    }
    __syncthreads();
    if constexpr (SMALL) {
#pragma unroll
        for (int q = 0; q < 2; ++q) {
            const int ch = tid + 256 * q;
            if (ch < c) {
                float acc = 0.f;
#pragma unroll
                for (int m = 0; m < MW2; ++m)
                    if (m < mid) acc += w2v[q][m] * hid[m];
                gate[ch] = 1.0f / (1.0f + expf(-acc));
            }
        }
    } else {
        for (int ch = tid; ch < c; ch += 256) {
            float acc = 0.f;
#pragma unroll 8
            for (int m = 0; m < mid; ++m) acc += w2[m * c + ch] * hid[m];
            gate[ch] = 1.0f / (1.0f + expf(-acc));
        }
    }
    __syncthreads();
    const int c4n = c >> 2;
    const long long base = ((long long)img * hw + (long long)blockIdx.x * rows) * c;
    const int total4 = rows * c4n;
    unsigned vm = 0u;
    for (int i = tid; i < total4; i += 256) {
        const int cc = i % c4n;
        const f32x4 yy = *(const f32x4*)(y + base + (long long)i * 4);
        const f32x4 rr = *(const f32x4*)(sc + base + (long long)i * 4);
        const f32x4 ss = *(const f32x4*)&gate[cc * 4];
        f32x4 o = ss * yy + rr;
        if (packed) vm = range_acc(range_acc(range_acc(range_acc(vm, o.x), o.y), o.z), o.w);
        o.x = fmaxf(o.x, 0.f); o.y = fmaxf(o.y, 0.f); o.z = fmaxf(o.z, 0.f); o.w = fmaxf(o.w, 0.f);
        if (out) *(f32x4*)(out + base + (long long)i * 4) = o;
        if (packed) {
            typedef _Float16 h4 __attribute__((ext_vector_type(4)));
            const h4 hi = {(_Float16)o.x, (_Float16)o.y, (_Float16)o.z, (_Float16)o.w};
            const h4 lo = {(_Float16)((o.x - (float)hi.x) * 2048.0f), (_Float16)((o.y - (float)hi.y) * 2048.0f),
                           (_Float16)((o.z - (float)hi.z) * 2048.0f), (_Float16)((o.w - (float)hi.w) * 2048.0f)};
            const long long pix = (long long)img * hw + (long long)blockIdx.x * rows + i / c4n;
            *(h4*)(packed + pix * 2 * c + cc * 4) = hi;
            *(h4*)(packed + pix * 2 * c + c + cc * 4) = lo;
        }
    }
    range_raise(fault, vm);
}

__global__ __launch_bounds__(256) void gem_neck_kernel(const float* __restrict__ x, int hw, int c,
                                                       const float* __restrict__ p_ptr, const float* __restrict__ scale,
                                                       const float* __restrict__ shift, float* __restrict__ gem_out,
                                                       float* __restrict__ emb, int* __restrict__ fault) {
    __shared__ float part[16][64 + 1];
    const int img = blockIdx.y, c0 = blockIdx.x * 64;
    const int quad = threadIdx.x & 15, pg = threadIdx.x >> 4;
    const float p = p_ptr[0];
    const bool cube = p == 3.0f;
    float acc[4] = {0.f, 0.f, 0.f, 0.f};
    const float* xi = x + (long long)img * hw * c + c0 + quad * 4;
    auto powp = [&](float f) {
        const float e = p * __builtin_amdgcn_logf(f);
        return e < -126.f ? __builtin_amdgcn_exp2f(e + 64.f) * 0x1p-64f : __builtin_amdgcn_exp2f(e);
    };
    int px = pg;
    for (; px + 7 * 16 < hw; px += 8 * 16) {
        f32x4 v[8];
#pragma unroll
        for (int u = 0; u < 8; ++u) v[u] = *(const f32x4*)(xi + (long long)(px + 16 * u) * c);
#pragma unroll
        for (int u = 0; u < 8; ++u)
#pragma unroll
            for (int e = 0; e < 4; ++e) {
                const float f = fmaxf(v[u][e], 1e-6f);
                acc[e] += cube ? f * f * f : powp(f);
            }
    }
    for (; px < hw; px += 16) {
        const f32x4 v = *(const f32x4*)(xi + (long long)px * c);
#pragma unroll
        for (int e = 0; e < 4; ++e) {
            const float f = fmaxf(v[e], 1e-6f);
            acc[e] += cube ? f * f * f : powp(f);
        }
    }
#pragma unroll
    for (int e = 0; e < 4; ++e) part[pg][quad * 4 + e] = acc[e];
    __syncthreads();
    if (threadIdx.x < 64) {
        float t = 0.f;
#pragma unroll
        for (int g = 0; g < 16; ++g) t += part[g][threadIdx.x];
        const int ch = c0 + threadIdx.x;
        const float m = t / (float)hw;
        const float g = cube ? cbrtf(m) : powf(m, 1.0f / p);
        if (gem_out) gem_out[(long long)img * c + ch] = g;
        const float ev = g * scale[ch] + shift[ch];
        emb[(long long)img * c + ch] = ev;
        if (fault && !(fabsf(ev) < INFINITY)) fault[1] = 1;
    }
}

__global__ __launch_bounds__(256) void row_sqnorm_kernel(const float* __restrict__ x, int m, int d, long long ld,
                                                         float* __restrict__ out) {
    const int row = blockIdx.x * 4 + (threadIdx.x >> 6), lane = threadIdx.x & 63;
    if (row >= m) return;
    const float* xr = x + (long long)row * ld;
    float acc = 0.f;
    for (int k = lane; k < d; k += 64) acc += xr[k] * xr[k];
    acc = wave_sum(acc);
    if (lane == 0) out[row] = acc;
}

inline int grid_for(long long work, int block) {
    long long g = (work + block - 1) / block;
    return (int)(g < 1 ? 1 : (g > 2048 ? 2048 : g));
}

}

int launch_nchw_to_nhwc3(reid_ctx* ctx, const float* x, int n, int h, int w, float* out) {
    const long long npix = (long long)n * h * w;
    prof_begin(ctx, REID_K_ELEMENTWISE, 0, npix * 24.0);
    hipLaunchKernelGGL(nchw_to_nhwc3_kernel, dim3(grid_for(npix, 256)), dim3(256), 0, ctx->stream, x, npix, h * w, out);
    prof_end(ctx);
    LAUNCH_CHECK();
    return REID_OK;
}

int launch_resize_norm(reid_ctx* ctx, const uint8_t* packed, const long long* offsets, const int* hw, int n, int H, int W,
                       int pitch, float* out) {
    const long long total = (long long)n * H * W;
    prof_begin(ctx, REID_K_ELEMENTWISE, 0, total * 15.0);
    hipLaunchKernelGGL(resize_norm_kernel, dim3(grid_for(total, 256)), dim3(256), 0, ctx->stream, packed, offsets, hw, n,
                       H, W, pitch, out);
    prof_end(ctx);
    LAUNCH_CHECK();
    return REID_OK;
}

int launch_maxpool3s2(reid_ctx* ctx, const float* x, int n, int h, int w, int c, float* out) {
    ARG_CHECK(c % 4 == 0);
    const int ho = (h + 2 - 3) / 2 + 1, wo = (w + 2 - 3) / 2 + 1;
    const long long total = (long long)n * ho * wo * (c / 4);
    prof_begin(ctx, REID_K_ELEMENTWISE, 0, ((double)n * h * w * c + (double)n * ho * wo * c) * 4.0);
    hipLaunchKernelGGL(maxpool3s2_kernel, dim3(grid_for(total, 256)), dim3(256), 0, ctx->stream, x, n, h, w, c, ho, wo, out);
    prof_end(ctx);
    LAUNCH_CHECK();
    return REID_OK;
}

int launch_norm_finalize(reid_ctx* ctx, const float* stats, int n_img, int tiles, int c, int half, int hw,
                         const float* in_gamma, const float* in_beta, const float* bn_scale, const float* bn_shift,
                         float* a_scale, float* a_shift) {
    prof_begin(ctx, REID_K_ELEMENTWISE, 0, (double)n_img * c * (tiles * 8.0 + 8.0));
    hipLaunchKernelGGL(norm_finalize_kernel, dim3(n_img), dim3(c < 256 ? c : 256), 0, ctx->stream, stats, tiles, c, half, hw,
                       in_gamma, in_beta, bn_scale, bn_shift, a_scale, a_shift);
    prof_end(ctx);
    LAUNCH_CHECK();
    return REID_OK;
}

int launch_in_apply(reid_ctx* ctx, float* x, const float* stats, int n_img, int tiles, int c, int half, int hw,
                    const float* in_gamma, const float* in_beta) {
    ARG_CHECK(half >= 4 && half % 4 == 0 && half <= 256 && hw % 128 == 0);
    prof_begin(ctx, REID_K_ELEMENTWISE, 0, (double)n_img * hw * half * 8.0);
    hipLaunchKernelGGL(in_apply_kernel, dim3(hw / 128, n_img), dim3(256), 0, ctx->stream, x, stats, tiles, c, half, hw, 128, in_gamma,
                       in_beta);
    prof_end(ctx);
    LAUNCH_CHECK();
    return REID_OK;
}

int launch_in_apply_pack(reid_ctx* ctx, const float* x, const float* stats, int n_img, int tiles, int c, int half, int hw,
                         const float* in_gamma, const float* in_beta, _Float16* packed, bool in_half_only) {
    ARG_CHECK(half >= 4 && half % 4 == 0 && c % 4 == 0 && c <= 512 && hw % 128 == 0 && packed);
    int rows = 128;
    while ((long long)n_img * (hw / rows) < 512 && rows > 16) rows >>= 1;
    prof_begin(ctx, REID_K_ELEMENTWISE, 0, (double)n_img * hw * (in_half_only ? half : c) * 8.0);
    hipLaunchKernelGGL(in_apply_pack_kernel, dim3(hw / rows, n_img), dim3(256), 0, ctx->stream, x, stats, tiles, c, half, hw, rows,
                       in_gamma, in_beta, packed, in_half_only ? 1 : 0, ctx->fault);
    prof_end(ctx);
    LAUNCH_CHECK();
    return REID_OK;
}

int launch_se_finalize(reid_ctx* ctx, const float* stats, int n_img, int tiles, int c, int mid, int hw, const float* w1,
                       const float* w2, float* s) {
    ARG_CHECK(c <= 512 && mid <= 64);
    prof_begin(ctx, REID_K_ELEMENTWISE, 0, (double)n_img * c * (tiles * 8.0 + 4.0));
    hipLaunchKernelGGL(se_finalize_kernel, dim3(n_img), dim3(256), 0, ctx->stream, stats, tiles, c, mid, hw, w1, w2, s);
    prof_end(ctx);
    LAUNCH_CHECK();
    return REID_OK;
}

int launch_se_combine(reid_ctx* ctx, const float* y, const float* sc, const float* s, int n_img, int hw, int c, float* out) {
    ARG_CHECK(c % 4 == 0);
    const long long total4 = (long long)n_img * hw * (c / 4);
    prof_begin(ctx, REID_K_ELEMENTWISE, 0, total4 * 48.0);
    hipLaunchKernelGGL(se_combine_kernel, dim3(grid_for(total4, 256)), dim3(256), 0, ctx->stream, y, sc, s, total4, hw, c, out);
    prof_end(ctx);
    LAUNCH_CHECK();
    return REID_OK;
}

int tail_slices(int n_img, int hw) {
    int s = 1;
    while ((long long)n_img * s < 1024 && hw / (s * 2) >= 16 && hw % (s * 2) == 0) s *= 2;
    return s;
}

int launch_se_tail(reid_ctx* ctx, const float* stats, int n_img, int tiles, int c, int mid, int hw, const float* w1, const float* w2,
                   const float* y, const float* sc, float* out, _Float16* packed) {
    return launch_se_tail_form(ctx, -1, stats, n_img, tiles, c, mid, hw, w1, w2, y, sc, out, packed);
}

int launch_se_tail_form(reid_ctx* ctx, int form, const float* stats, int n_img, int tiles, int c, int mid, int hw, const float* w1,
                        const float* w2, const float* y, const float* sc, float* out, _Float16* packed) {
    ARG_CHECK(c % 4 == 0 && c <= 512 && mid <= 64 && (out || packed) && form >= -1 && form <= 1 && (form != 1 || mid <= 32));
    const int slices = tail_slices(n_img, hw);
    prof_begin(ctx, REID_K_ELEMENTWISE, 0, (double)n_img * hw * c * 12.0);
    if (form < 0 ? (long long)slices * n_img <= 512 && c >= 512 && mid <= 32 : form == 1)
        hipLaunchKernelGGL(se_tail_kernel<true>, dim3(slices, n_img), dim3(256), 0, ctx->stream, stats, tiles, c, mid, hw, w1, w2, y, sc,
                           hw / slices, out, packed, ctx->fault);
    else
        hipLaunchKernelGGL(se_tail_kernel<false>, dim3(slices, n_img), dim3(256), 0, ctx->stream, stats, tiles, c, mid, hw, w1, w2, y, sc,
                           hw / slices, out, packed, ctx->fault);
    prof_end(ctx);
    LAUNCH_CHECK();
    return REID_OK;
}

int launch_gem_neck(reid_ctx* ctx, const float* x, int n_img, int hw, int c, const float* p, const float* scale,
                    const float* shift, float* gem_out, float* emb) {
    ARG_CHECK(c % 64 == 0);
    prof_begin(ctx, REID_K_ELEMENTWISE, 0, (double)n_img * hw * c * 4.0);
    hipLaunchKernelGGL(gem_neck_kernel, dim3(c / 64, n_img), dim3(256), 0, ctx->stream, x, hw, c, p, scale, shift, gem_out, emb,
                       ctx->fault);
    prof_end(ctx);
    LAUNCH_CHECK();
    return REID_OK;
}

int launch_row_sqnorm(reid_ctx* ctx, const float* x, int m, int d, long long ld, float* out) {
    prof_begin(ctx, REID_K_ELEMENTWISE, 0, (double)m * d * 4.0);
    hipLaunchKernelGGL(row_sqnorm_kernel, dim3((m + 3) / 4), dim3(256), 0, ctx->stream, x, m, d, ld, out);
    prof_end(ctx);
    LAUNCH_CHECK();
    return REID_OK;
}

namespace {
__global__ void add_indexed_rows_kernel(float* __restrict__ x, long long per_img, int C, const float* __restrict__ table,
                                        const int32_t* __restrict__ idx, float coeff) {
    const int img = blockIdx.y;
    const float* row = table + (long long)idx[img] * C;
    float* xi = x + (long long)img * per_img;
    for (long long i = (long long)blockIdx.x * blockDim.x + threadIdx.x; i < per_img; i += (long long)gridDim.x * blockDim.x)
        xi[i] += coeff * row[i % C];
}
}

int launch_add_indexed_rows(reid_ctx* ctx, float* x, int n, long long hw, int C, const float* table, const int32_t* d_idx, float coeff) {
    ARG_CHECK(x && table && d_idx && n >= 1 && hw >= 1 && C >= 1);
    const long long per_img = hw * C;
    const int gx = (int)((per_img + 256 * 8 - 1) / (256 * 8));
    prof_begin(ctx, REID_K_ELEMENTWISE, (double)n * per_img * 2.0, (double)n * per_img * 8.0);
    hipLaunchKernelGGL(add_indexed_rows_kernel, dim3(gx < 1 ? 1 : gx, n), dim3(256), 0, ctx->stream, x, per_img, C, table, d_idx, coeff);
    prof_end(ctx);
    LAUNCH_CHECK();
    return REID_OK;
}
```

### real-time-reid-tracking_amd/csrc/reid_internal.h

```cpp
#pragma once
#include <hip/hip_runtime.h>
#include <stdint.h>
#include <stddef.h>
#include <stdio.h>
#include <string>
#include <map>
#include <tuple>
#include <vector>
#include "../../include/reid_hip.h"
struct reid_ctx;

void reid_set_error(const char* fmt, ...);

#define HIP_TRY(expr)                                                                         \
    do {                                                                                      \
        hipError_t _e = (expr);                                                               \
        if (_e != hipSuccess) {                                                               \
            reid_set_error("%s:%d %s -> %s", __FILE__, __LINE__, #expr, hipGetErrorString(_e)); \
            return REID_ERR_HIP;                                                              \
        }                                                                                     \
    } while (0)

#define REID_TRY(expr)            \
    do {                          \
// ... 88 lines not shown
    const float* col_scale;
    const float* col_shift;
    const _Float16* residual;
    int relu;
    float* stats;
    const _Float16* zero_page;
    unsigned long long* diag;
    int lin, act, n_real;
    int asym, pad_y, pad_x;
    int scat_h, scat_w, scat_py, scat_px;
    float* C32;
    const float* res32;
    unsigned scat_mhw, scat_mw;
    int par4;
    long long par_stride;
    int split_k;
    float* splitk_ws;
    int* splitk_cnt;
    _Float16* pack16;
    int pack_from;
    int loader_prio;
    int frag_ahead;
    float acc_scale;
    int relu_from;
    int split_terms;
    int pack_out;
    int a_k;
    int pair_early;
    int general_epi;
    int ablate;
    int* fault;
};

__device__ __forceinline__ float l2sqr_of(float dot, float rs, float cq) { return fmaf(-2.0f, dot, rs + cq); }

__device__ __forceinline__ unsigned range_acc(unsigned m, float v) {
    const unsigned b = __float_as_uint(v) & 0x7fffffffu;
    return b > m ? b : m;
}
__device__ __forceinline__ void range_raise(int* fault, unsigned m) {
    if (fault && m >= 0x477fe000u) fault[0] = 1;
}

template <class P>
inline void set_scatter(P& p, int scat_h, int scat_w, int py, int px) {
    p.scat_h = scat_h; p.scat_w = scat_w; p.scat_py = py; p.scat_px = px;
    p.scat_mhw = p.scat_mw = 0;
    if (scat_h > 0) {
        p.scat_mhw = (unsigned)(((1ull << 32) + (unsigned long long)(scat_h * scat_w) - 1) / (unsigned long long)(scat_h * scat_w));
        p.scat_mw = (unsigned)(((1ull << 32) + (unsigned long long)scat_w - 1) / (unsigned long long)scat_w);
    }
}

struct reid_ctx;
int launch_gemm_f16(reid_ctx* ctx, int amode, const Gemm16Params& p, int kind, double flops, double bytes);
bool conv3x3_f16_supported(const Gemm16Params& p);
int launch_conv3x3_f16(reid_ctx* ctx, const Gemm16Params& p, int kind, double flops, double bytes);
int launch_conv3x3_split(reid_ctx* ctx, const Gemm16Params& p, int kind, double flops, double bytes);
bool conv3x3_x3_supported(const reid_ctx* ctx, const Gemm16Params& p);
int launch_conv3x3_x3(reid_ctx* ctx, const Gemm16Params& p);
bool lin_x3_supported(const reid_ctx* ctx, const Gemm16Params& p);
int launch_lin_x3(reid_ctx* ctx, const Gemm16Params& p, int kind, double flops, double bytes);
bool conv_x3s_supported(const reid_ctx* ctx, const Gemm16Params& p);
int launch_conv_x3s(reid_ctx* ctx, const Gemm16Params& p, int kind, double flops, double bytes);
int launch_gemm_f16_split(reid_ctx* ctx, const Gemm16Params& p, int kind, double flops, double bytes);
bool two_linear_supported(const reid_ctx*, long long T, int C, int hid);
int launch_two_linear(reid_ctx*, const _Float16* a16, long long T, int C, int hid, const float* w1, const float* b1, const float* w2,
                      const float* b2, int act, const float* res, float* out, const float* x32 = nullptr, const float* ln_g = nullptr,
                      const float* ln_b = nullptr);
bool ln_linear_supported(const reid_ctx*, long long T, int C, int n);
int launch_ln_linear(reid_ctx*, const float* x32, const float* ln_g, const float* ln_b, long long T, int C, int n, const float* w, const float* bias,
                     float* out, int ldc);
int launch_window_attn_cos(reid_ctx* ctx, int mode, const void* qkv, int ldq, int n_img, int H, int W, int heads, int shifted,
                           const float* bias_t, const float* scale, void* out);
int launch_post_norm(reid_ctx* ctx, int side_mode, const float* x, const float* y, long long T, int C, const float* g, const float* b,
                     float* out, _Float16* side);
void swin_bias_table(const float* pos169, float* tab4096);
int swin_attn_ldq(const reid_ctx* ctx, int C);
int launch_window_attn(reid_ctx* ctx, const void* qkv, int n, int Hs, int Ws, int heads, int shifted, const float* pos, const float* bias_tab,
                       void* out);
int launch_swin_layernorm(reid_ctx* ctx, int form, const float* x, long long T, int C, const float* g, const float* b, void* out);
int launch_sfe_norm_fc(reid_ctx* ctx, const float* c1, int n, int h1, int w1, const float* in_g, const float* in_b, const float* bn_s,
                       const float* bn_t, const float* c2_w, const float* c2_b, const float* fc_w, const float* fc_b, float* ab, float* tok);
int launch_swin_tail(reid_ctx* ctx, const float* x, int n, int ntok, const float* g, const float* b, const float* p, const float* bn_s,
                     const float* bn_t, float* gem, float* emb);
int swin_loaded_merge(reid_ctx* ctx, int stage, const float* x, int n, int h, int w, float* scratch, float* out);
int swin_loaded_fuse(reid_ctx* ctx, const float* sfe, float* const* xs, int n, int h1, int w1, float* scratch16, float* a0, float* f3, float* f2,
                     float* f1);
int launch_sfe_conv1(reid_ctx* ctx, const float* x, int n, int h, int w, const float* c1_w, const float* c1_b, float* c1);
int swin_crops_check(int out_h, int out_w, const float* mean_std6);
int launch_swin_crop_front(reid_ctx* ctx, const uint8_t* d_src, const long long* d_off, const int* d_hw, int n, int h, int w, int pitch,
                           const float* mean_std6, const float* c1_w, const float* c1_b, float* c1);
int launch_split_pack(reid_ctx* ctx, const float* x, long long rows, int C, _Float16* out, const float* d_scale = nullptr);
int launch_split_weights(reid_ctx* ctx, const float* w, int cout, int taps, int cin, int terms, _Float16* out, const float* d_scale = nullptr);
int launch_prep_u8_pad_f16(reid_ctx*, const uint8_t* crops, int n, int h, int w, int hp, int wp, _Float16* out);
int launch_prep_f32_pad_f16(reid_ctx*, const float* nhwc3, int n, int h, int w, int hp, int wp, _Float16* out);
int launch_maxpool3s2_f16(reid_ctx*, const _Float16* x, int n, int h, int w, int c, _Float16* out);
int launch_affine_relu_f16(reid_ctx*, _Float16* x, const float* a_scale, const float* a_shift, int n_img, int hw, int c);
int launch_norm_apply_f16(reid_ctx*, _Float16* x, const float* stats, int n_img, int tiles, int c, int half, int hw,
                          const float* in_gamma, const float* in_beta, const float* bn_scale, const float* bn_shift);
int launch_se_tail_f16(reid_ctx*, const float* stats, int n_img, int tiles, int c, int mid, int hw, const float* w1, const float* w2t,
                       const _Float16* y, const _Float16* sc, _Float16* out);
int launch_se_combine_f16(reid_ctx*, const _Float16* y, const _Float16* sc, const float* s, int n_img, int hw, int c,
                          _Float16* out);
int launch_gem_neck_f16(reid_ctx*, const _Float16* x, int n_img, int hw, int c, const float* p, const float* scale,
                        const float* shift, float* gem_out, float* emb);
int launch_f32_to_f16(reid_ctx*, const float* x, size_t n, _Float16* out);
int launch_stem_w16(reid_ctx*, const float* stem_w_f32, _Float16* out);
bool conv3x3_c64_f16_supported(int H, int W, int Cin, int Cout, int R, int S, int stride, int pad);
int launch_scale_rows_f16(reid_ctx*, const float* w, const float* scale, int rows, int k, _Float16* out);
int launch_conv3x3_c64_f16(reid_ctx*, const _Float16* in, int n, const _Float16* w_scaled, const float* shift,
                           const _Float16* residual, int relu, float* stats, _Float16* out, const _Float16* zero_page,
                           const float* se_w1 = nullptr, const float* se_w2t = nullptr);
int launch_stem_w16_scaled(reid_ctx*, const float* stem_w_f32, const float* scale, _Float16* out);
int launch_stem_pool_f16(reid_ctx*, const _Float16* pad_in, const uint8_t* crops_u8, int n, const _Float16* w16s, const float* shift,
                         _Float16* pooled);
int launch_conv_w16_chunked(reid_ctx*, const float* w_f32, int cout, int rs, int cin, _Float16* out);
int launch_gemm_f32(reid_ctx* ctx, int amode, int epi, const GemmParams& p, int kind, double flops, double bytes);
int launch_ta_tail(reid_ctx* ctx, const float* y, const float* sc, int n_img, int H, int W, int C, const float* wts, float* out);
int launch_ema_tail(reid_ctx* ctx, const float* y, const float* sc, int n_img, int H, int W, int C, const float* prm, float* out);
int launch_stem_split(reid_ctx* ctx, const void* x, bool is_u8, int n, const float* wgt, const float* scale, const float* shift, float* out,
                      _Float16* packed);
int launch_stem_f32(reid_ctx* ctx, const void* x, bool is_u8, int n, const float* wgt, const float* scale, const float* shift,
                    float* out, bool pooled);
bool gemm_f32_dma_supported(int amode, int epi, const GemmParams& p);
int launch_gemm_f32_dma(reid_ctx* ctx, int epi, const GemmParams& p, int kind, double flops, double bytes);
bool conv_f32_supported(const GemmParams& p);
int launch_conv_f32(reid_ctx* ctx, const GemmParams& p, int kind, double flops, double bytes);
bool conv_f32_general_supported(const GemmParams& p);
int launch_conv_f32_general(reid_ctx* ctx, const GemmParams& p, int kind, double flops, double bytes);

int launch_nchw_to_nhwc3(reid_ctx*, const float* x_nchw, int n, int h, int w, float* out_nhwc);
int launch_resize_norm(reid_ctx*, const uint8_t* packed, const long long* offsets, const int* hw, int n, int H, int W,
                       int pitch, float* out_nhwc);
int launch_maxpool3s2(reid_ctx*, const float* x, int n, int h, int w, int c, float* out);
int launch_norm_finalize(reid_ctx*, const float* stats, int n_img, int tiles, int c, int half, int hw,
                         const float* in_gamma, const float* in_beta, const float* bn_scale, const float* bn_shift,
                         float* a_scale, float* a_shift);
int launch_in_apply(reid_ctx*, float* x, const float* stats, int n_img, int tiles, int c, int half, int hw, const float* in_gamma,
                    const float* in_beta);
int launch_se_finalize(reid_ctx*, const float* stats, int n_img, int tiles, int c, int mid, int hw, const float* w1,
                       const float* w2, float* s);
int tail_slices(int n_img, int hw);
int launch_se_tail(reid_ctx*, const float* stats, int n_img, int tiles, int c, int mid, int hw, const float* w1, const float* w2,
                   const float* y, const float* sc, float* out, _Float16* packed = nullptr);
int launch_se_tail_form(reid_ctx*, int form, const float* stats, int n_img, int tiles, int c, int mid, int hw, const float* w1,
                        const float* w2, const float* y, const float* sc, float* out, _Float16* packed);
int launch_se_combine(reid_ctx*, const float* y, const float* sc, const float* s, int n_img, int hw, int c, float* out);
int launch_in_apply_pack(reid_ctx*, const float* x, const float* stats, int n_img, int tiles, int c, int half, int hw,
                         const float* in_gamma, const float* in_beta, _Float16* packed,
                         bool in_half_only = false);
int launch_gem_neck(reid_ctx*, const float* x, int n_img, int hw, int c, const float* p, const float* scale,
                    const float* shift, float* gem_out, float* emb);
int launch_row_sqnorm(reid_ctx*, const float* x, int m, int d, long long ld, float* out);
int launch_argmin_rows(reid_ctx*, const float* dist, int m, int n, long long ld, int32_t* idx, float* val);
int launch_topk_rows(reid_ctx*, const float* dist, int m, int n, long long ld, int k, float* D, int32_t* I);
int launch_rank_eval(reid_ctx*, const float* score, int nq, int ng, long long ld, const long long* ql,
                     const long long* qc, const long long* gl, const long long* gc, int32_t* cmc_sum, double* ap,
                     int32_t* valid);
int launch_diou_cost(reid_ctx*, const double* tracks, int t, const double* dets, int m, double* out, int as_cost);

struct ProfSlot {
    double ms = 0, flops = 0, bytes = 0;
    long long launches = 0;
};

struct Se18Block {
    int c, cin, stride, ibn, ds, mid;
    const float *conv1_w, *in_gamma, *in_beta, *bn1_scale, *bn1_shift, *conv2_w, *bn2_scale, *bn2_shift;
    const float *ds_w, *ds_scale, *ds_shift, *se_w1, *se_w2;
    const float *ta, *ema;
};

struct Se18Weights {
    bool loaded = false;
    float* blob = nullptr;
    size_t n_floats = 0;
    int num_class = 0;
    int arch = 0;
    const float *stem_w, *stem_scale, *stem_shift;
    Se18Block blk[8];
    const float *gem_p, *neck_scale, *neck_shift, *cls_w;
    const float* cam_bias = nullptr;
    int num_cams = 0;
    float cam_factor = -1.0f;
    _Float16* blob16 = nullptr;
    _Float16* stem_w16 = nullptr;
    _Float16* l1_conv2_w16s[2] = {nullptr, nullptr};
    _Float16* stem_w16s = nullptr;
    _Float16* zero_page = nullptr;
    float* ep = nullptr;
    const _Float16* h(const float* p) const { return blob16 + (p - blob); }
};

struct reid_comm_loop {
    virtual int allgather(int rank, const void* d_send, void* d_recv, size_t bytes, hipStream_t st) = 0;
    virtual int allreduce(int rank, double* inout, int count, int op) = 0;
    virtual void detach(int rank) = 0;
    virtual ~reid_comm_loop() {}
};
struct reid_comm {
    void* comm = nullptr;
    int rank = 0, world = 1;
    reid_comm_loop* loop = nullptr;
};
void comm_release(reid_ctx* ctx);
int launch_knn_merge(reid_ctx* ctx, const float* Dall, const int32_t* Iall, int world, int nq, int kk, int k, float* D, int32_t* I);

struct reid_ctx {
    int device = 0;
    reid_comm* comm = nullptr;
    hipStream_t stream = nullptr;
    hipStream_t own_stream = nullptr;
    int chunk = 1024;
    int precision = 0;
    bool profile = false;
    ProfSlot prof[REID_K_COUNT];
    std::vector<std::pair<hipEvent_t, hipEvent_t>> ev_pool;
    struct Pending { int kind; hipEvent_t a, b; double flops, bytes; };
    std::vector<Pending> pending;
    hipEvent_t t0 = nullptr, t1 = nullptr;
    std::map<std::string, std::pair<void*, size_t>> ws;
    std::map<std::string, std::pair<void*, size_t>> pinned;
    std::map<const void*, void*> split_w;
    int bank_fast = 1;
    Se18Weights se18;
    int last_n = 0;
    int swin_last_n = 0, swin_last_tok = 0;
    int debug_keep = 0;
    bool last_f16 = false;
    int f16_wide_splitk = 1;
    int f16_frag_ahead = 1;
    int f16_loader_prio = 1;
    int f16_loader_waves = 1;
    int f16_halo = 1;
    int f16_se_tail = 1;
    int f16_c64 = 2;
    int f16_stem_fused = 2;
    int f32_conv = 1;
    int f32_split_k = 1;
    int lin_x3 = 1;
    int f32_dist_bk16 = 1;
    int pack_epilogue = 1;
    int split_lean_epi = 1;
    int split_x3 = 3;
    int split_gemm_min_tiles = 128;
    int chain = 0;
    int x3_sk_cap = 0;
    int split_x3_small = 2;
    int x3s_sk_cap = 8;
    int conv_x3s = 1;
    int x3_l4_narrow_nmt = 31;
    int x3_narrow = 1;
    int x3_unroll = 3;
    int x3_ablate = 0;
    int split_x3_min_blocks = 512;
    int split_pair = 0;
    int stem_split = 1;
    int f32_stem_pool = 1;
    int split_terms = 3;
    int knn_wide = 1;
    long long knn_wide_min = 1ll << 25;
    int knn_wide_force = 0;
    int select_exp = 0;
    int select_two_pass = 0;
    int rerank_hbm_acc = 0;
    int swin_stop = -1;
    int swin_fold = 1;
    int swin_two_linear = 1;
    int swin_attn_split = 0;
    int two_linear_ablate = 0;
    int swin_attn_mfma = 1;
    int f16_split_k = 1;
    int swin_chunk_cap = 1024;
    int f16_lin_256 = 1;
    int f16_cfg = 0;
    int frame_m[2] = {0, 0};
    float* frame_emb[2] = {nullptr, nullptr};
    int frame_pending[2] = {0, 0}, frame_has[2] = {0, 0};
    size_t frame_tm[2] = {0, 0};
    hipEvent_t frame_ev[2] = {nullptr, nullptr};
    hipStream_t match_stream = nullptr;
    int match_async = 0;
    hipEvent_t join_ev = nullptr;
    hipEvent_t fwd_ev[2] = {nullptr, nullptr}, match_ev[2] = {nullptr, nullptr};
    hipStream_t copy_stream = nullptr;
    hipEvent_t copy_ev = nullptr;
    std::vector<hipEvent_t> pipe_ev;
    int host_pipeline = 1;
    int side_copy = 1;
    std::vector<int32_t> side_idx;
    size_t side_cursor = 0;
    const char* frame_out[2] = {nullptr, nullptr};
    float* stage_ptr[11] = {nullptr};
    unsigned long long* conv_diag = nullptr;
    std::string split_bad_se18, split_bad_swin;
    int* fault = nullptr;
};
enum { REID_FAULT_RANGE = 1, REID_FAULT_NONFINITE = 2 };
int ctx_fault_status(reid_ctx* ctx);
bool knn_wide_eligible(reid_ctx* ctx, int nq, int nb, int d, int k);
int knn_wide_dev(reid_ctx* ctx, const float* xp, int nq, const float* yp, int nb, int ld, const float* rs, const float* cq, int k, float* d_D,
                 int32_t* d_I);

inline std::string split_range_violation(const float* blob, const std::map<std::string, std::pair<size_t, size_t>>& tab,
                                         const std::vector<std::pair<std::string, float>>& suffix_bound) {
    for (const auto& kv : tab) {
        for (const auto& sb : suffix_bound) {
            const std::string& suf = sb.first;
            if (kv.first.size() < suf.size() || kv.first.compare(kv.first.size() - suf.size(), suf.size(), suf) != 0) continue;
            float mx = 0.f;
            const float* w = blob + kv.second.first;
            for (size_t i = 0; i < kv.second.second; ++i) {
                const float a = w[i] < 0 ? -w[i] : w[i];
                if (!(a <= mx)) mx = a;
            }
            if (!(mx < sb.second)) {
                char buf[160];
                snprintf(buf, sizeof(buf), "%s (max |w| = %g, limit %g)", kv.first.c_str(), (double)mx, (double)sb.second);
                return buf;
            }
            break;
        }
    }
    return std::string();
}

struct ChainElem {
    const float* x;
    const float* stats;
    const float* sc;
    const float *g, *b;
    float* out;
    _Float16* packed;
    int c, half, hw, tiles, mid, slices;
};
struct ChainStage {
    int kind;
    int idx;
    int first, items;
    int dep;
    int target;
    int sk;
};
struct ChainParams {
    int n_img, n_stages, total_items, flags;
    ChainStage st[8];
    Gemm16Params conv[4];
    ChainElem el[4];
    int* counters;
    int* fault;
};
int launch_chain(reid_ctx* ctx, const ChainParams& cp, int W);

int conv_gemm(reid_ctx* ctx, int amode, const void* x, int n, int H, int W, int Cin, const float* wgt, int Cout, int R,
              int S, int stride, int pad, int Kpad, const float* a_scale, const float* a_shift, int a_relu,
              const float* col_scale, const float* col_shift, const float* residual, int relu, float* stats, float* out,
              int relu_from = 0, const _Float16* x_packed = nullptr,
              _Float16* out_packed = nullptr, int pack_from = 0, bool* packed_written = nullptr);
int conv_weights_fresh(reid_ctx* ctx, const float* d_w);
int conv_weights_splittable(reid_ctx* ctx, const float* h_w, size_t count, const char* who);
int conv_gemm16(reid_ctx* ctx, int amode, const _Float16* x, int n, int H, int W, int Cin, const _Float16* wgt, int Cout,
                int R, int S, int stride, int pad, int K, const float* col_scale, const float* col_shift,
                const _Float16* residual, int relu, float* stats, _Float16* out, int Hp = 0, int Wp = 0);

struct DeviceGuard {
    int prev = -1, dev = -1;
    explicit DeviceGuard(int d) : dev(d) {
        if (hipGetDevice(&prev) != hipSuccess) prev = -1;
        if (prev != dev) (void)hipSetDevice(dev);
    }
    ~DeviceGuard() {
        if (prev >= 0 && prev != dev) (void)hipSetDevice(prev);
    }
    DeviceGuard(const DeviceGuard&) = delete;
    DeviceGuard& operator=(const DeviceGuard&) = delete;
};
#define CTX_GUARD(ctx) DeviceGuard _dev_guard((ctx)->device)
#define CTX_ENTER(ctx)            \
    CTX_GUARD(ctx);               \
    REID_TRY(ctx_fault_status(ctx))

void swin_release(reid_ctx* ctx);
int ctx_ws(reid_ctx* ctx, const char* name, size_t bytes, void** out);
int ctx_take_side(reid_ctx* ctx, int n, int rows, const char* what, const int32_t** d_idx);
int launch_add_indexed_rows(reid_ctx* ctx, float* x, int n, long long hw, int C, const float* table, const int32_t* d_idx, float coeff);
int ctx_pinned(reid_ctx* ctx, const char* name, size_t bytes, void** out);
int ctx_pipe_events(reid_ctx* ctx, int passes);
// ... 62 lines not shown
```

### real-time-reid-tracking_amd/engine.py

```python
import ctypes as C

import numpy as np

from . import _ffi
from ._ffi import check

_ENGINES = {}

IMG_H, IMG_W = 256, 128


def _f32(a):
    return np.ascontiguousarray(a, dtype=np.float32)


def _ptr(a):
    return a.ctypes.data_as(C.c_void_p) if a is not None else None


class Engine:
    def __init__(self, device=0):
        self.lib = _ffi.lib()
        h = C.c_void_p()
        check(self.lib.reid_ctx_create(int(device), C.byref(h)))
# ... 333 lines not shown
        sl = np.ascontiguousarray(np.concatenate(sl), np.int32) if sl else None
        tb = np.ascontiguousarray(np.concatenate(tb)) if boxes else None
        db = np.ascontiguousarray(np.concatenate(db)) if boxes else None
        check(self.lib.reid_frame_cost_groups(self.h, int(slot), k, banks if sl is not None else None, _ptr(tc), _ptr(mc), _ptr(sl), int(metric),
                                              C.c_float(max_dist), _ptr(tb), _ptr(db), 1 if want_emb else 0))
        tm = int((tc.astype(np.int64) * mc).sum())
        self.__dict__.setdefault("_frame_q", {})[slot] = (self._frame_n[slot], tm, want_emb, sl is not None and tm > 0, boxes and tm > 0, tc, mc)

    def frame_fetch_groups(self, slot):
        m, tm, want_emb, has_cost, has_iou, tc, mc = self._frame_q.pop(slot)
        emb = np.empty((m, 512), np.float32) if want_emb else None
        cost = np.empty(tm, np.float32) if has_cost else None
        iou = np.empty(tm, np.float64) if has_iou else None
        check(self.lib.reid_frame_fetch(self.h, int(slot), _ptr(emb) if m else None, _ptr(cost), _ptr(iou)))
        offs = np.concatenate([[0], np.cumsum(tc.astype(np.int64) * mc)])
        cut = lambda a: [None if a is None else a[offs[g]:offs[g + 1]].reshape(int(tc[g]), int(mc[g])) for g in range(len(tc))]
        return emb, cut(cost), cut(iou)

    def frame_update(self, slot, bank, rows, slots):
        rows = np.ascontiguousarray(rows, np.int32)
        slots = np.ascontiguousarray(slots, np.int32)
        check(self.lib.reid_frame_update(self.h, int(slot), bank, _ptr(rows), _ptr(slots), len(rows)))

    def embed_frame_u8(self, frame, boxes_xyxy, logits=False):
        frame = np.ascontiguousarray(frame, dtype=np.uint8)
        if frame.ndim != 3 or frame.shape[2] != 3:
            raise ValueError("frame must be uint8[H,W,3], got %s" % (frame.shape,))
        boxes = np.ascontiguousarray(boxes_xyxy, dtype=np.int32).reshape(-1, 4)
        n = boxes.shape[0]
        emb, lg = self._outs(n, logits)
        check(self.lib.reid_embed_frame_u8(self.h, _ptr(frame), frame.shape[0], frame.shape[1], _ptr(boxes), n, _ptr(emb),
                                           _ptr(lg)))
        return (emb, lg) if logits else emb

    def embed_f32_nchw(self, x, logits=False):
        x = _f32(x)
        if x.ndim != 4 or x.shape[1:] != (3, IMG_H, IMG_W):
            raise ValueError("embed_f32_nchw expects float32[n,3,%d,%d], got %s" % (IMG_H, IMG_W, x.shape))
        emb, lg = self._outs(x.shape[0], logits)
        check(self.lib.reid_embed_f32_nchw(self.h, _ptr(x), x.shape[0], _ptr(emb), _ptr(lg)))
        return (emb, lg) if logits else emb

    def embed_f32_nchw_dev(self, d_x, n, d_emb, d_logits=None):
        check(self.lib.reid_embed_f32_nchw_dev(self.h, C.c_void_p(d_x), int(n), C.c_void_p(d_emb), C.c_void_p(d_logits or 0)))

    def embed_u8_dev(self, d_crops, n, d_emb, d_logits=None):
        check(self.lib.reid_embed_u8_dev(self.h, C.c_void_p(d_crops), int(n), C.c_void_p(d_emb),
                                         C.c_void_p(d_logits or 0)))

    def debug_switch(self, name, value=None):
        dbg = _ffi.debug_lib()
        if value is None:
            v = C.c_longlong()
            check(dbg.reid_debug_get_switch(self.h, name.encode(), C.byref(v)))
            return v.value
        check(dbg.reid_debug_set_switch(self.h, name.encode(), C.c_longlong(int(value))))

    def debug_mfma_bare(self, shape, zero=False, iters=20000):
        tf = C.c_float()
        check(_ffi.debug_lib().reid_debug_mfma_bare(self.h, int(shape), int(bool(zero)), int(iters), C.byref(tf)))
        return tf.value

    def debug_switches_from_env(self):
        import os
        spec = os.environ.get("REID_DEBUG_SWITCHES", "")
        for item in filter(None, (t.strip() for t in spec.split(","))):
            name, _, val = item.partition("=")
            self.debug_switch(name.strip(), int(val))
        return spec

    def debug_keep(self, on):
        check(self.lib.reid_ctx_set_debug_keep(self.h, int(on)))

    def debug_stage(self, stage, n):
        sizes = [524288, 131072, 131072, 131072, 65536, 65536, 32768, 32768, 65536, 65536, 512]
        out = np.empty(sizes[stage] * n, np.float32)
        cnt = C.c_size_t()
        check(self.lib.reid_debug_stage(self.h, int(stage), _ptr(out), out.size, C.byref(cnt)))
        assert cnt.value == out.size
        return out

    def debug_conv_layer(self, x, w, stride=1, pad=0, scale=None, shift=None, residual=None, relu=False, relu_from=0, pack_from=-1,
                         stats=False, a_scale=None, a_shift=None, a_relu=False):
        x, w = _f32(x), _f32(w)
        n, h, ww, cin = x.shape
        cout, r, s, wc = w.shape
        if r != s or wc != cin:
            raise ValueError("debug_conv_layer expects w[cout, r, r, cin] matching x")
        ho, wo = (h + 2 * pad - r) // stride + 1, (ww + 2 * pad - r) // stride + 1
        m = n * ho * wo
        out = np.empty((n, ho, wo, cout), np.float32)
        pk = np.empty((m, 2 * cout), np.uint16) if pack_from >= 0 else None
        st = np.empty((m // 128, cout, 2), np.float32) if stats else None
        opt = [_f32(a) if a is not None else None for a in (scale, shift, residual, a_scale, a_shift)]
        written = C.c_int(0)
        check(_ffi.debug_lib().reid_debug_conv_layer(
            self.h, _ptr(x), C.c_int(n), C.c_int(h), C.c_int(ww), C.c_int(cin), _ptr(w), C.c_int(cout), C.c_int(r), C.c_int(stride),
            C.c_int(pad), _ptr(opt[0]), _ptr(opt[1]), _ptr(opt[2]), C.c_int(int(bool(relu))), C.c_int(int(relu_from)),
            C.c_int(int(pack_from)), C.c_int(int(bool(stats))), _ptr(opt[3]), _ptr(opt[4]), C.c_int(int(bool(a_relu))), _ptr(out),
            _ptr(pk), _ptr(st), C.byref(written)))
        return out, (pk if written.value else None), st

    def debug_norm_finish(self, form, x, stats, in_gamma, in_beta, bn_scale=None, bn_shift=None, hw=None):
        stats = _f32(stats)
        n, tiles, c, _ = stats.shape
        half = int(np.asarray(in_gamma).size)
        hw = int(hw) if x is None else x.shape[1]
        xa = None if form == 0 else (np.ascontiguousarray(x, np.uint16) if form >= 4 else _f32(x))
        out = np.empty((n, hw, c), np.float32) if 1 <= form <= 3 else None
        o16 = np.empty((n * hw, 2 * c), np.uint16) if form in (2, 3) else (np.empty((n, hw, c), np.uint16) if form >= 4 else None)
        ab = [np.empty((n, c), np.float32) for _ in range(2)] if form in (0, 5) else [None, None]
        opt = [_f32(a) if a is not None else None for a in (in_gamma, in_beta, bn_scale, bn_shift)]
        check(_ffi.debug_lib().reid_debug_norm_finish(
            self.h, C.c_int(form), C.c_int(n), C.c_int(hw), C.c_int(c), C.c_int(half), C.c_int(tiles), _ptr(xa), _ptr(stats),
            _ptr(opt[0]), _ptr(opt[1]), _ptr(opt[2]), _ptr(opt[3]), _ptr(out), _ptr(o16), _ptr(ab[0]), _ptr(ab[1])))
        return out, o16, ab[0], ab[1]

    def debug_se_tail(self, form, stats, w1, w2t, y, shortcut):
        stats = _f32(stats)
        n, tiles, c, _ = stats.shape
        mid = w1.shape[0]
        hw = y.shape[1]
        f16 = form >= 10
        cv = (lambda a: np.ascontiguousarray(a, np.uint16)) if f16 else _f32
        ya, sa = cv(y), cv(shortcut)
        tail = 1 <= form <= 9
        want_out = not f16 and (not tail or (form - 1) % 3 != 1)
        want_pk = tail and (form - 1) % 3 != 0
        out = np.empty((n, hw, c), np.float32) if want_out else None
        o16 = np.empty((n, hw, c), np.uint16) if f16 else (np.empty((n * hw, 2 * c), np.uint16) if want_pk else None)
        gate = np.empty((n, c), np.float32) if form in (0, 11) else None
        check(_ffi.debug_lib().reid_debug_se_tail(
            self.h, C.c_int(form), C.c_int(n), C.c_int(hw), C.c_int(c), C.c_int(mid), C.c_int(tiles), _ptr(stats), _ptr(_f32(w1)),
            _ptr(_f32(w2t)), _ptr(ya), _ptr(sa), _ptr(out), _ptr(o16), _ptr(gate)))
        return out, o16, gate

    def debug_sibling_tail(self, arch, prm, y, shortcut):
        y, shortcut = _f32(y), _f32(shortcut)
        n, h, w, c = y.shape
        out = np.empty((n, h, w, c), np.float32)
        check(_ffi.debug_lib().reid_debug_sibling_tail(self.h, C.c_int(arch), C.c_int(n), C.c_int(h), C.c_int(w), C.c_int(c), _ptr(_f32(prm)),
                                                       _ptr(y), _ptr(shortcut), _ptr(out)))
        return out

    def debug_gem_neck(self, x, p, scale, shift, f16=False):
        x = np.ascontiguousarray(x, np.uint16) if f16 else _f32(x)
        n, hw, c = x.shape
        g, e = np.empty((n, c), np.float32), np.empty((n, c), np.float32)
        check(_ffi.debug_lib().reid_debug_gem_neck(
            self.h, C.c_int(int(bool(f16))), C.c_int(n), C.c_int(hw), C.c_int(c), C.c_float(p), _ptr(x), _ptr(_f32(scale)),
            _ptr(_f32(shift)), _ptr(g), _ptr(e)))
        return g, e

    def debug_stem(self, form, x, w, scale, shift):
        is_u8 = np.asarray(x).dtype == np.uint8
        x = np.ascontiguousarray(x, np.uint8) if is_u8 else _f32(x)
        n = x.shape[0]
        if x.shape[1:] != (IMG_H, IMG_W, 3) or np.shape(w) != (64, 7, 7, 3):
            raise ValueError("debug_stem expects x[n, 256, 128, 3] and w[64, 7, 7, 3]")
        out = np.empty((n, 128, 64, 64) if form == 0 else (n, 64, 32, 64), np.float32) if form in (0, 1, 2, 6) else None
        o16 = np.empty((n * 2048, 128), np.uint16) if form == 2 else (np.empty((n, 64, 32, 64), np.uint16) if form in (3, 4, 5) else None)
        check(_ffi.debug_lib().reid_debug_stem(self.h, C.c_int(form), C.c_int(int(is_u8)), _ptr(x), C.c_int(n), _ptr(_f32(w)),
                                               _ptr(_f32(scale)), _ptr(_f32(shift)), _ptr(out), _ptr(o16)))
        return out, o16

    def debug_resize_norm(self, packed, offsets, hw, pitch=0):
        packed = np.ascontiguousarray(packed, np.uint8).reshape(-1)
        offsets = np.ascontiguousarray(offsets, np.int64)
        hw = np.ascontiguousarray(hw, np.int32).reshape(-1, 2)
        n = len(offsets)
        end = max(int(o) + ((int(h) - 1) * (pitch or int(w)) + int(w)) * 3 for o, (h, w) in zip(offsets, hw))
        if len(hw) != n or end > packed.size:
            raise ValueError("debug_resize_norm: a window leaves the buffer")
        out = np.empty((n, IMG_H, IMG_W, 3), np.float32)
        check(_ffi.debug_lib().reid_debug_resize_norm(self.h, _ptr(packed), _ptr(offsets), _ptr(hw), C.c_int(n), C.c_int(int(pitch)), _ptr(out)))
        return out

    def debug_swin_crop_front(self, packed, offsets, hw, c1_w, c1_b, size=(224, 224), mean_std=None, pitch=0):
        h_out, w_out, ms = self._swin_crop_args(size, mean_std)
        if ms is None:
            ms = _f32([0.485, 0.456, 0.406, 0.229, 0.224, 0.225])
        packed = np.ascontiguousarray(packed, np.uint8).reshape(-1)
        offsets = np.ascontiguousarray(offsets, np.int64)
        hw = np.ascontiguousarray(hw, np.int32).reshape(-1, 2)
        n = len(offsets)
        end = max(int(o) + ((int(h) - 1) * (pitch or int(w)) + int(w)) * 3 for o, (h, w) in zip(offsets, hw))
        if len(hw) != n or end > packed.size or int(offsets.min()) < 0 or int(hw.min()) < 1:
            raise ValueError("debug_swin_crop_front: a window leaves the buffer")
        c1_w, c1_b = _f32(c1_w).reshape(-1), _f32(c1_b).reshape(-1)
        if c1_w.size != 144 or c1_b.size != 12:
            raise ValueError("debug_swin_crop_front expects c1_w[12,2,2,3] and c1_b[12]")
        out = np.empty((n, h_out // 2, w_out // 2, 12), np.float32)
        check(_ffi.debug_lib().reid_debug_swin_crop_front(self.h, _ptr(packed), _ptr(offsets), _ptr(hw), C.c_int(n), C.c_int(int(pitch)),
                                                          C.c_int(h_out), C.c_int(w_out), _ptr(ms), _ptr(c1_w), _ptr(c1_b), _ptr(out)))
        return out

    def debug_swin_conv1(self, x, c1_w, c1_b):
        x, c1_w, c1_b = _f32(x), _f32(c1_w).reshape(-1), _f32(c1_b).reshape(-1)
        n, c, h, w = x.shape
        if c != 3 or h % 2 or w % 2 or c1_w.size != 144 or c1_b.size != 12:
            raise ValueError("debug_swin_conv1 expects x[n,3,2k,2m], c1_w[12,2,2,3] and c1_b[12]")
        out = np.empty((n, h // 2, w // 2, 12), np.float32)
        check(_ffi.debug_lib().reid_debug_swin_conv1(self.h, _ptr(x), C.c_int(n), C.c_int(h), C.c_int(w), _ptr(c1_w), _ptr(c1_b), _ptr(out)))
        return out

    def debug_maxpool(self, x):
        f16 = np.asarray(x).dtype == np.uint16
        x = np.ascontiguousarray(x, np.uint16) if f16 else _f32(x)
        n, h, w, c = x.shape
        out = np.empty((n, (h - 1) // 2 + 1, (w - 1) // 2 + 1, c), x.dtype)
        check(_ffi.debug_lib().reid_debug_maxpool(self.h, C.c_int(int(f16)), _ptr(x), C.c_int(n), C.c_int(h), C.c_int(w), C.c_int(c), _ptr(out)))
        return out

    def debug_window_attn_cos(self, mode, qkv, bias, scale, shifted):
        qkv, bias, scale = _f32(qkv), _f32(bias), _f32(scale)
        n, h, w, c3 = qkv.shape
        heads = bias.shape[0]
        assert c3 == 3 * heads * 32 and bias.shape == (heads, 49, 49) and scale.shape == (heads,)
        c = heads * 32
        out = np.empty((n, h, w, c), np.float32) if mode == 0 else None
        o16 = None if mode == 0 else np.empty((n * h * w, 2 * c if mode == 2 else c), np.uint16)
        check(_ffi.debug_lib().reid_debug_window_attn_cos(
            self.h, C.c_int(mode), _ptr(qkv), C.c_int(n), C.c_int(h), C.c_int(w), C.c_int(heads), C.c_int(int(bool(shifted))), _ptr(bias),
            _ptr(scale), _ptr(out), _ptr(o16)))
        if mode == 0:
            return out
        f = o16.view(np.float16)
        if mode == 2:
            return (f[:, :c].astype(np.float64) + f[:, c:].astype(np.float64) / 2048.0).reshape(n, h, w, c)
        return f.astype(np.float32).reshape(n, h, w, c)

    def debug_post_norm(self, side, x, y, g, b, in_place=False):
        x, y = _f32(x), _f32(y)
        t, c = x.shape
        out = np.empty((t, c), np.float32)
        o16 = None if side == 0 else np.empty((t, 2 * c if side == 2 else c), np.uint16)
        check(_ffi.debug_lib().reid_debug_post_norm(
            self.h, C.c_int(side), _ptr(x), _ptr(y), C.c_int(t), C.c_int(c), _ptr(_f32(g)), _ptr(_f32(b)), C.c_int(int(bool(in_place))),
            _ptr(out), _ptr(o16)))
        if side == 0:
            return out, None
        f = o16.view(np.float16)
        return out, (f[:, :c].astype(np.float64) + f[:, c:].astype(np.float64) / 2048.0) if side == 2 else f.astype(np.float32)

    @staticmethod
    def _unpack16(o16, c):
        f = o16.view(np.float16)
        return f[:, :c].astype(np.float64) + f[:, c:].astype(np.float64) / 2048.0

    def debug_window_attn(self, form, qkv, pos, shifted, raw=False):
        qkv, pos = _f32(qkv), _f32(pos).reshape(-1)
        n, h, w, c3 = qkv.shape
        c = c3 // 3
        if c3 != 3 * c or c % 32 or pos.size != 169:
            raise ValueError("debug_window_attn expects qkv[n, h, w, 3 * heads * 32] and pos[13, 13]")
        out = np.empty((n, h, w, c), np.float32) if form in (0, 5) else None
        o16 = None if form in (0, 5) else np.empty((n * h * w, 2 * c if form in (1, 4) else c), np.uint16)
        check(_ffi.debug_lib().reid_debug_window_attn(
            self.h, C.c_int(form), _ptr(qkv), C.c_int(n), C.c_int(h), C.c_int(w), C.c_int(c // 32), C.c_int(int(bool(shifted))), _ptr(pos),
            _ptr(out), _ptr(o16)))
        if raw:
            return out if o16 is None else o16
        if o16 is None:
            return out
        if form in (1, 4):
            return self._unpack16(o16, c).reshape(n, h, w, c)
        return o16.view(np.float16).astype(np.float32).reshape(n, h, w, c)

    def debug_layernorm(self, form, x, g, b):
        x = _f32(x)
        t, c = x.shape
        out = np.empty((t, c), np.float32) if form == 0 else None
        o16 = None if form == 0 else np.empty((t, 2 * c if form == 2 else c), np.uint16)
        check(_ffi.debug_lib().reid_debug_layernorm(self.h, C.c_int(form), _ptr(x), C.c_int(t), C.c_int(c), _ptr(_f32(g)), _ptr(_f32(b)),
                                                    _ptr(out), _ptr(o16)))
        return out if form == 0 else o16

    def debug_ln_linear(self, x, ln_g, ln_b, w, bias=None):
        x, w = _f32(x), _f32(w)
        t, c = x.shape
        n = w.shape[0]
        out = np.empty((t, n), np.float32)
        check(_ffi.debug_lib().reid_debug_ln_linear(self.h, _ptr(x), _ptr(_f32(ln_g)), _ptr(_f32(ln_b)), _ptr(w),
                                                    _ptr(_f32(bias) if bias is not None else None), C.c_int(t), C.c_int(c), C.c_int(n), _ptr(out)))
        return out

    def debug_swin_sfe(self, c1, in_g, in_b, bn_s, bn_t, c2_w, c2_b, fc_w, fc_b):
        c1 = _f32(c1)
        n, h1, w1, _ = c1.shape
        prm = [_f32(a).reshape(-1) for a in (in_g, in_b, bn_s, bn_t, c2_w, c2_b, fc_w, fc_b)]
        if c1.shape[3] != 12 or [a.size for a in prm] != [6, 6, 6, 6, 2304, 48, 4608, 96]:
            raise ValueError("debug_swin_sfe: operand shapes")
        ab, tok = np.empty((n, 24), np.float32), np.empty((n, h1 // 2, w1 // 2, 96), np.float32)
        check(_ffi.debug_lib().reid_debug_swin_sfe(self.h, _ptr(c1), C.c_int(n), C.c_int(h1), C.c_int(w1), *[_ptr(a) for a in prm], _ptr(ab),
                                                   _ptr(tok)))
        return ab, tok

    def debug_swin_tail(self, x, g, b, p, bn_s, bn_t):
        x = _f32(x)
        n, ntok, c = x.shape
        prm = [_f32(a).reshape(-1) for a in (g, b, bn_s, bn_t)]
        if c != 96 or any(a.size != 96 for a in prm):
            raise ValueError("debug_swin_tail expects x[n, ntok, 96] and 96-channel parameters")
        gem, emb = np.empty((n, 96), np.float32), np.empty((n, 96), np.float32)
        check(_ffi.debug_lib().reid_debug_swin_tail(self.h, _ptr(x), C.c_int(n), C.c_int(ntok), _ptr(prm[0]), _ptr(prm[1]), C.c_float(p),
                                                    _ptr(prm[2]), _ptr(prm[3]), _ptr(gem), _ptr(emb)))
# ... 189 lines not shown
```

Measured before the change: 84100 crops/s.

## Fuse final SE tail into GeM pooling neck kernel for last block

For the last ResNet block, the SE gate computation, gated residual add with ReLU, and GeM pooling plus BN neck now run in one kernel instead of an SE-tail kernel followed by a separate GeM kernel. This avoids writing the block output to memory and reading it back. The per-image gate is recomputed by each block in the grid, and the channel loop is strided. The norm-finish kernel also gets batched tile-sum reduction and a strided, unrolled pack loop. The fused path is gated by a minimum batch threshold.

```diff
diff --git a/include/reid_hip_debug.h b/include/reid_hip_debug.h
--- a/include/reid_hip_debug.h
+++ b/include/reid_hip_debug.h
@@ -32,6 +32,9 @@
                             float* out);
 int reid_debug_gem_neck(reid_ctx* ctx, int f16, int n, int hw, int c, float p, const void* x, const float* scale, const float* shift,
                         float* gem_out, float* emb);
+int reid_debug_gem_neck_fused(reid_ctx* ctx, int n, int hw, int c, int mid, int tiles, float p, const float* stats, const float* w1,
+                              const float* w2t, const float* y, const float* shortcut, const float* scale, const float* shift,
+                              float* gem_out, float* emb);
 int reid_debug_stem(reid_ctx* ctx, int form, int is_u8, const void* x, int n, const float* w, const float* scale, const float* shift,
                     float* out, uint16_t* out16);
 int reid_debug_resize_norm(reid_ctx* ctx, const uint8_t* packed, const long long* offsets, const int* hw, int n, int pitch, float* out);
diff --git a/real-time-reid-tracking_amd/_ffi.py b/real-time-reid-tracking_amd/_ffi.py
--- a/real-time-reid-tracking_amd/_ffi.py
+++ b/real-time-reid-tracking_amd/_ffi.py
@@ -102,7 +102,7 @@
 
 DEBUG_LIB_PATH = os.path.join(_HERE, "libreid_hip_debug.so")
 DEBUG_EXPORTS = ("reid_debug_coissue", "reid_debug_comm_loopback", "reid_debug_conv_c64", "reid_debug_conv_layer", "reid_debug_conv_split", "reid_debug_conv_diag", "reid_debug_conv_f16", "reid_debug_conv_f32",
-                 "reid_debug_feed", "reid_debug_gem_neck", "reid_debug_gemm_f16", "reid_debug_knn_merge", "reid_debug_knn_wide", "reid_debug_layernorm", "reid_debug_linear", "reid_debug_linear_rows", "reid_debug_ln_linear", "reid_debug_maxpool", "reid_debug_mfma_bare", "reid_debug_mfma_shape", "reid_debug_norm_finish", "reid_debug_post_norm", "reid_debug_resize_norm", "reid_debug_se_tail", "reid_debug_stem", "reid_debug_sibling_tail", "reid_debug_swin_conv1", "reid_debug_swin_crop_front", "reid_debug_swin_fuse", "reid_debug_swin_merge", "reid_debug_swin_sfe", "reid_debug_swin_tail", "reid_debug_select_exp", "reid_debug_set_switch", "reid_debug_get_switch", "reid_debug_two_linear", "reid_debug_two_linear_ablate", "reid_debug_window_attn", "reid_debug_window_attn_cos")
+                 "reid_debug_feed", "reid_debug_gem_neck", "reid_debug_gem_neck_fused", "reid_debug_gemm_f16", "reid_debug_knn_merge", "reid_debug_knn_wide", "reid_debug_layernorm", "reid_debug_linear", "reid_debug_linear_rows", "reid_debug_ln_linear", "reid_debug_maxpool", "reid_debug_mfma_bare", "reid_debug_mfma_shape", "reid_debug_norm_finish", "reid_debug_post_norm", "reid_debug_resize_norm", "reid_debug_se_tail", "reid_debug_stem", "reid_debug_sibling_tail", "reid_debug_swin_conv1", "reid_debug_swin_crop_front", "reid_debug_swin_fuse", "reid_debug_swin_merge", "reid_debug_swin_sfe", "reid_debug_swin_tail", "reid_debug_select_exp", "reid_debug_set_switch", "reid_debug_get_switch", "reid_debug_two_linear", "reid_debug_two_linear_ablate", "reid_debug_window_attn", "reid_debug_window_attn_cos")
 
 _lib = None
 _dbg = None
diff --git a/real-time-reid-tracking_amd/csrc/api.hip b/real-time-reid-tracking_amd/csrc/api.hip
--- a/real-time-reid-tracking_amd/csrc/api.hip
+++ b/real-time-reid-tracking_amd/csrc/api.hip
@@ -812,6 +812,7 @@
 
     const float* cur = b.pool;
     int H = 64, W = 32;
+    bool gem_done = false;
     if (split_mode && !stem_split) REID_TRY(launch_split_pack(ctx, b.pool, (long long)n * 64 * 32, 64, cur16));
     for (int i = 0; i < 8; ++i) {
         const Se18Block& k = w.blk[i];
@@ -890,8 +891,14 @@
                 fp32_read = !(conv_split_path(ctx, n, Ho, Wo, nx.cin, nx.c, 3, 3, nx.stride, 1) &&
                               conv_split_path(ctx, n, Ho, Wo, nx.cin, nx.c, 1, 1, nx.stride, 0));
             }
-            REID_TRY(launch_se_tail(ctx, b.stats, n, tiles, k.c, k.mid, hw, k.se_w1, k.se_w2, y, shortcut, fp32_read ? out : nullptr,
-                                    i < 7 ? cur16 : nullptr));
+            if (i == 7 && !keep && n >= ctx->gem_tail_min) {
+                REID_TRY(launch_gem_neck_tail(ctx, b.stats, n, tiles, k.c, k.mid, hw, k.se_w1, k.se_w2, y, shortcut, w.gem_p, w.neck_scale,
+                                              w.neck_shift, b.gem, d_emb));
+                gem_done = true;
+            } else {
+                REID_TRY(launch_se_tail(ctx, b.stats, n, tiles, k.c, k.mid, hw, k.se_w1, k.se_w2, y, shortcut, fp32_read ? out : nullptr,
+                                        i < 7 ? cur16 : nullptr));
+            }
         } else {
             REID_TRY(launch_se_finalize(ctx, b.stats, n, tiles, k.c, k.mid, hw, k.se_w1, k.se_w2, b.se));
             REID_TRY(launch_se_combine(ctx, y, shortcut, b.se, n, hw, k.c, out));
@@ -901,7 +908,7 @@
         H = Ho;
         W = Wo;
     }
-    REID_TRY(launch_gem_neck(ctx, cur, n, H * W, 512, w.gem_p, w.neck_scale, w.neck_shift, b.gem, d_emb));
+    if (!gem_done) REID_TRY(launch_gem_neck(ctx, cur, n, H * W, 512, w.gem_p, w.neck_scale, w.neck_shift, b.gem, d_emb));
     {
         const int32_t* d_cam;
         REID_TRY(ctx_take_side(ctx, n, w.num_cams, "reid_embed (camera bias)", &d_cam));
diff --git a/real-time-reid-tracking_amd/csrc/debug.hip b/real-time-reid-tracking_amd/csrc/debug.hip
--- a/real-time-reid-tracking_amd/csrc/debug.hip
+++ b/real-time-reid-tracking_amd/csrc/debug.hip
@@ -18,7 +18,7 @@
     {"f16_se_tail", &reid_ctx::f16_se_tail}, {"f16_c64", &reid_ctx::f16_c64}, {"swin_chunk_cap", &reid_ctx::swin_chunk_cap},
     {"split_x3", &reid_ctx::split_x3}, {"x3_ablate", &reid_ctx::x3_ablate}, {"x3_unroll", &reid_ctx::x3_unroll}, {"x3_narrow", &reid_ctx::x3_narrow}, {"conv_x3s", &reid_ctx::conv_x3s}, {"x3s_sk_cap", &reid_ctx::x3s_sk_cap}, {"x3_l4_narrow_nmt", &reid_ctx::x3_l4_narrow_nmt}, {"split_x3_small", &reid_ctx::split_x3_small}, {"split_x3_min_blocks", &reid_ctx::split_x3_min_blocks}, {"f32_dist_bk16", &reid_ctx::f32_dist_bk16}, {"lin_x3", &reid_ctx::lin_x3},
     {"host_pipeline", &reid_ctx::host_pipeline}, {"x3_sk_cap", &reid_ctx::x3_sk_cap}, {"chain", &reid_ctx::chain}, {"split_gemm_min_tiles", &reid_ctx::split_gemm_min_tiles},
-    {"rerank_hbm_acc", &reid_ctx::rerank_hbm_acc},
+    {"rerank_hbm_acc", &reid_ctx::rerank_hbm_acc}, {"gem_tail_min", &reid_ctx::gem_tail_min},
 };
 }
 
@@ -634,6 +634,30 @@
     return ctx_fault_status(ctx);
 }
 
+extern "C" int reid_debug_gem_neck_fused(reid_ctx* ctx, int n, int hw, int c, int mid, int tiles, float p, const float* stats, const float* w1,
+                                         const float* w2t, const float* y, const float* shortcut, const float* scale, const float* shift,
+                                         float* gem_out, float* emb) {
+    ARG_CHECK(ctx && n >= 1 && hw >= 1 && c >= 64 && mid >= 1 && tiles >= 1 && stats && w1 && w2t && y && shortcut && scale && shift && emb);
+    CTX_ENTER(ctx);
+    const size_t ny = (size_t)n * hw * c, ne = (size_t)n * c;
+    float *dst, *dw1, *dw2, *dy, *dsc, *dp, *dbs, *dbh, *dg = nullptr, *de;
+    REID_TRY(dbg_upload(ctx, "dbgt.stats", stats, (size_t)n * tiles * c * 2, &dst));
+    REID_TRY(dbg_upload(ctx, "dbgt.w1", w1, (size_t)mid * c, &dw1));
+    REID_TRY(dbg_upload(ctx, "dbgt.w2", w2t, (size_t)mid * c, &dw2));
+    REID_TRY(dbg_upload(ctx, "dbgt.x", y, ny, &dy));
+    REID_TRY(dbg_upload(ctx, "dbgt.sc", shortcut, ny, &dsc));
+    REID_TRY(dbg_upload(ctx, "dbgt.p", &p, 1, &dp));
+    REID_TRY(dbg_upload(ctx, "dbgt.bns", scale, (size_t)c, &dbs));
+    REID_TRY(dbg_upload(ctx, "dbgt.bnh", shift, (size_t)c, &dbh));
+    if (gem_out) REID_TRY(dbg_output(ctx, "dbgt.a", ne, &dg));
+    REID_TRY(dbg_output(ctx, "dbgt.b", ne, &de));
+    REID_TRY(launch_gem_neck_tail(ctx, dst, n, tiles, c, mid, hw, dw1, dw2, dy, dsc, dp, dbs, dbh, dg, de));
+    if (dg) REID_TRY(dbg_download(ctx, gem_out, dg, ne));
+    REID_TRY(dbg_download(ctx, emb, de, ne));
+    HIP_TRY(hipStreamSynchronize(ctx->stream));
+    return ctx_fault_status(ctx);
+}
+
 extern "C" int reid_debug_two_linear_ablate(reid_ctx* ctx, int bits) {
     ARG_CHECK(ctx && bits >= 0 && bits < 4);
     ctx->two_linear_ablate = bits;
diff --git a/real-time-reid-tracking_amd/csrc/elementwise.hip b/real-time-reid-tracking_amd/csrc/elementwise.hip
--- a/real-time-reid-tracking_amd/csrc/elementwise.hip
+++ b/real-time-reid-tracking_amd/csrc/elementwise.hip
@@ -14,6 +14,40 @@
 #pragma unroll
     for (int o = 32; o > 0; o >>= 1) v += __shfl_xor(v, o);
     return v;
+}
+
+template <int NV, int B>
+__device__ __forceinline__ void tile_batch(const float* __restrict__ st, int& t, int c, double (&s)[NV]) {
+    float v[B][NV];
+#pragma unroll
+    for (int u = 0; u < B; ++u)
+#pragma unroll
+        for (int k = 0; k < NV; ++k) v[u][k] = st[(long long)(t + u) * c * 2 + k];
+#pragma unroll
+    for (int u = 0; u < B; ++u)
+#pragma unroll
+        for (int k = 0; k < NV; ++k) s[k] += (double)v[u][k];
+    t += B;
+}
+template <int NV>
+__device__ __forceinline__ void tile_sums(const float* __restrict__ st, int tiles, int c, double (&s)[NV]) {
+#pragma unroll
+    for (int k = 0; k < NV; ++k) s[k] = 0.0;
+    int t = 0;
+    while (tiles - t >= 16) tile_batch<NV, 16>(st, t, c, s);
+    if (tiles - t >= 8) tile_batch<NV, 8>(st, t, c, s);
+    if (tiles - t >= 4) tile_batch<NV, 4>(st, t, c, s);
+    if (tiles - t >= 2) tile_batch<NV, 2>(st, t, c, s);
+    if (tiles - t >= 1) tile_batch<NV, 1>(st, t, c, s);
+}
+
+typedef _Float16 h4 __attribute__((ext_vector_type(4)));
+__device__ __forceinline__ void store_pair(_Float16* __restrict__ p, int c, const f32x4 v) {
+    const h4 hi = {(_Float16)v.x, (_Float16)v.y, (_Float16)v.z, (_Float16)v.w};
+    const h4 lo = {(_Float16)((v.x - (float)hi.x) * 2048.0f), (_Float16)((v.y - (float)hi.y) * 2048.0f),
+                   (_Float16)((v.z - (float)hi.z) * 2048.0f), (_Float16)((v.w - (float)hi.w) * 2048.0f)};
+    *(h4*)p = hi;
+    *(h4*)(p + c) = lo;
 }
 
 __global__ void nchw_to_nhwc3_kernel(const float* __restrict__ x, long long npix, int hw, float* __restrict__ out) {
@@ -172,40 +206,55 @@
             sb[ch] = 0.f;
             continue;
         }
-        double s1 = 0.0, s2 = 0.0;
-        for (int t = 0; t < tiles; ++t) {
-            const float* st = stats + (((long long)img * tiles + t) * c + ch) * 2;
-            s1 += (double)st[0];
-            s2 += (double)st[1];
-        }
-        const double mean = s1 / hw;
-        double var = s2 / hw - mean * mean;
+        const float g = in_gamma[ch], be = in_beta[ch];
+        double s12[2];
+        tile_sums<2>(stats + ((long long)img * tiles * c + ch) * 2, tiles, c, s12);
+        const double mean = s12[0] / hw;
+        double var = s12[1] / hw - mean * mean;
         if (var < 0.0) var = 0.0;
         const double inv = 1.0 / sqrt(var + 1e-5);
-        sa[ch] = (float)(inv * (double)in_gamma[ch]);
-        sb[ch] = (float)((double)in_beta[ch] - mean * inv * (double)in_gamma[ch]);
+        sa[ch] = (float)(inv * (double)g);
+        sb[ch] = (float)((double)be - mean * inv * (double)g);
     }
     __syncthreads();
     const int q = (in_only ? half : c) >> 2;
     const long long pix0 = (long long)img * hw + (long long)blockIdx.x * rows;
-    typedef _Float16 h4 __attribute__((ext_vector_type(4)));
+    const int total = rows * q;
     unsigned vm = 0u;
-    for (int i = tid; i < rows * q; i += 256) {
-        const int row = i / q, cc = i - row * q;
-        f32x4 v = *(const f32x4*)(x + (pix0 + row) * c + cc * 4);
-        if (cc * 4 < half) {
-            const f32x4 a = *(const f32x4*)&sa[cc * 4], b = *(const f32x4*)&sb[cc * 4];
-            v = v * a + b;
-            vm = range_acc(range_acc(range_acc(range_acc(vm, v.x), v.y), v.z), v.w);
-            v.x = fmaxf(v.x, 0.f); v.y = fmaxf(v.y, 0.f); v.z = fmaxf(v.z, 0.f); v.w = fmaxf(v.w, 0.f);
-        } else {
-            vm = range_acc(range_acc(range_acc(range_acc(vm, v.x), v.y), v.z), v.w);
-        }
-        const h4 hi = {(_Float16)v.x, (_Float16)v.y, (_Float16)v.z, (_Float16)v.w};
-        const h4 lo = {(_Float16)((v.x - (float)hi.x) * 2048.0f), (_Float16)((v.y - (float)hi.y) * 2048.0f),
-                       (_Float16)((v.z - (float)hi.z) * 2048.0f), (_Float16)((v.w - (float)hi.w) * 2048.0f)};
-        *(h4*)(packed + (pix0 + row) * 2 * c + cc * 4) = hi;
-        *(h4*)(packed + (pix0 + row) * 2 * c + c + cc * 4) = lo;
+    auto finish = [&](f32x4 v, bool inorm, const f32x4 a, const f32x4 b, _Float16* dst) {
+        if (inorm) v = v * a + b;
+        vm = range_acc(range_acc(range_acc(range_acc(vm, v.x), v.y), v.z), v.w);
+        if (inorm) { v.x = fmaxf(v.x, 0.f); v.y = fmaxf(v.y, 0.f); v.z = fmaxf(v.z, 0.f); v.w = fmaxf(v.w, 0.f); }
+        store_pair(dst, c, v);
+    };
+    if (256 % q == 0) {
+        const int cc = tid % q, rstep = 256 / q;
+        const bool inorm = cc * 4 < half;
+        const f32x4 a = *(const f32x4*)&sa[cc * 4], b = *(const f32x4*)&sb[cc * 4];
+        const float* xp = x + (pix0 + tid / q) * c + cc * 4;
+        _Float16* pp = packed + (pix0 + tid / q) * 2 * c + cc * 4;
+        const long long xs = (long long)rstep * c, ps = 2 * xs;
+        int i = tid;
+        for (; i + 3 * 256 < total; i += 4 * 256) {
+            f32x4 v[4];
+#pragma unroll
+            for (int u = 0; u < 4; ++u) v[u] = *(const f32x4*)(xp + u * xs);
+#pragma unroll
+            for (int u = 0; u < 4; ++u) finish(v[u], inorm, a, b, pp + u * ps);
+            xp += 4 * xs;
+            pp += 4 * ps;
+        }
+        for (; i < total; i += 256) {
+            finish(*(const f32x4*)xp, inorm, a, b, pp);
+            xp += xs;
+            pp += ps;
+        }
+    } else {
+        for (int i = tid; i < total; i += 256) {
+            const int row = i / q, cc = i - row * q;
+            const f32x4 v = *(const f32x4*)(x + (pix0 + row) * c + cc * 4);
+            finish(v, cc * 4 < half, *(const f32x4*)&sa[cc * 4], *(const f32x4*)&sb[cc * 4], packed + (pix0 + row) * 2 * c + cc * 4);
+        }
     }
     range_raise(fault, vm);
 }
@@ -253,6 +302,102 @@
 }
 
 template <bool SMALL>
+__device__ __forceinline__ void se_gate(const float* __restrict__ stats, int tiles, int c, int mid, int hw, const float* __restrict__ w1,
+                                        const float* __restrict__ w2, int img, float* pooled, float* hid, float* gate) {
+    const int tid = threadIdx.x, lane = tid & 63, wave = __builtin_amdgcn_readfirstlane(tid >> 6);
+    constexpr int MJ = SMALL ? 8 : 16, MW2 = 32;
+    constexpr int W1PRE = SMALL ? 8 : 4;
+    const int c4v = c >> 2;
+    f32x4 w1v[W1PRE][2];
+    float w2v[SMALL ? 2 : 1][SMALL ? MW2 : 1];
+#pragma unroll
+    for (int j = 0; j < W1PRE; ++j)
+#pragma unroll
+        for (int k = 0; k < 2; ++k)
+            w1v[j][k] = *(const f32x4*)(w1 + (long long)min(wave + 4 * j, mid - 1) * c + min(lane + 64 * k, c4v - 1) * 4);
+    if constexpr (SMALL) {
+#pragma unroll
+        for (int q = 0; q < 2; ++q)
+#pragma unroll
+            for (int m = 0; m < MW2; ++m) {
+                const int ch = tid + 256 * q;
+                if (ch < c && m < mid) w2v[q][m] = w2[m * c + ch];
+            }
+    }
+    for (int ch = tid; ch < c; ch += 256) {
+        double acc[1];
+        tile_sums<1>(stats + ((long long)img * tiles * c + ch) * 2, tiles, c, acc);
+        pooled[ch] = (float)(acc[0] / hw);
+    }
+    __syncthreads();
+    {
+        float acc[16];
+#pragma unroll
+        for (int j = 0; j < 16; ++j) acc[j] = 0.f;
+#pragma unroll
+        for (int g = 0; g < MJ / 4; ++g) {
+            if (wave + 16 * g >= mid) break;
+            f32x4 wg[4][2];
+#pragma unroll
+            for (int jj = 0; jj < 4; ++jj)
+#pragma unroll
+                for (int k = 0; k < 2; ++k) {
+                    const int j = 4 * g + jj, m = wave + 4 * j, c4 = lane + 64 * k;
+                    if (j < W1PRE) wg[jj][k] = w1v[j < W1PRE ? j : 0][k];
+                    else wg[jj][k] = *(const f32x4*)(w1 + (long long)min(m, mid - 1) * c + min(c4, c4v - 1) * 4);
+                }
+#pragma unroll
+            for (int jj = 0; jj < 4; ++jj)
+#pragma unroll
+                for (int k = 0; k < 2; ++k) {
+                    const int j = 4 * g + jj, m = wave + 4 * j, c4 = lane + 64 * k;
+                    if (m < mid && c4 < c4v) {
+                        const f32x4 wv = wg[jj][k];
+                        const f32x4 pv = *(const f32x4*)(pooled + c4 * 4);
+                        acc[j] += wv.x * pv.x + wv.y * pv.y + wv.z * pv.z + wv.w * pv.w;
+                    }
+                }
+        }
+#pragma unroll
+        for (int j = 0; j < 16; ++j) {
+            if (wave + 4 * j < mid) {
+                const float v = wave_sum(acc[j]);
+                if (lane == 0) hid[wave + 4 * j] = fmaxf(v, 0.f);
+            }
+        }
+    }
+    __syncthreads();
+    if constexpr (SMALL) {
+#pragma unroll
+        for (int q = 0; q < 2; ++q) {
+            const int ch = tid + 256 * q;
+            if (ch < c) {
+                float acc = 0.f;
+#pragma unroll
+                for (int m = 0; m < MW2; ++m)
+                    if (m < mid) acc += w2v[q][m] * hid[m];
+                gate[ch] = 1.0f / (1.0f + expf(-acc));
+            }
+        }
+    } else {
+        for (int ch = tid; ch < c; ch += 256) {
+            float acc = 0.f;
+            for (int m0 = 0; m0 < mid; m0 += 8) {
+                float wv[8];
+#pragma unroll
+                for (int u = 0; u < 8; ++u)
+                    if (m0 + u < mid) wv[u] = w2[(m0 + u) * c + ch];
+#pragma unroll
+                for (int u = 0; u < 8; ++u)
+                    if (m0 + u < mid) acc += wv[u] * hid[m0 + u];
+            }
+            gate[ch] = 1.0f / (1.0f + expf(-acc));
+        }
+    }
+    __syncthreads();
+}
+
+template <bool SMALL>
 __global__ __launch_bounds__(256) void se_tail_kernel(const float* __restrict__ stats, int tiles, int c, int mid, int hw,
                                                       const float* __restrict__ w1, const float* __restrict__ w2,
                                                       const float* __restrict__ y, const float* __restrict__ sc, int rows,
@@ -260,159 +405,137 @@
     __shared__ __attribute__((aligned(16))) float pooled[512];
     __shared__ float hid[64];
     __shared__ __attribute__((aligned(16))) float gate[512];
-    const int img = blockIdx.y, tid = threadIdx.x, lane = tid & 63, wave = tid >> 6;
-    constexpr int MJ = SMALL ? 8 : 16, MW2 = 32;
-    f32x4 w1v[SMALL ? 8 : 1][2];
-    float w2v[SMALL ? 2 : 1][SMALL ? MW2 : 1];
-    if constexpr (SMALL) {
-        const int c4v = c >> 2;
-#pragma unroll
-        for (int j = 0; j < MJ; ++j)
-#pragma unroll
-            for (int k = 0; k < 2; ++k) {
-                const int m = wave + 4 * j, c4 = lane + 64 * k;
-                if (m < mid && c4 < c4v) w1v[j][k] = *(const f32x4*)(w1 + (long long)m * c + c4 * 4);
-            }
-#pragma unroll
-        for (int q = 0; q < 2; ++q)
-#pragma unroll
-            for (int m = 0; m < MW2; ++m) {
-                const int ch = tid + 256 * q;
-                if (ch < c && m < mid) w2v[q][m] = w2[m * c + ch];
-            }
-    }
-    for (int ch = tid; ch < c; ch += 256) {
-        double acc = 0.0;
-        for (int t = 0; t < tiles; ++t) acc += (double)stats[(((long long)img * tiles + t) * c + ch) * 2];
-        pooled[ch] = (float)(acc / hw);
-    }
-    __syncthreads();
-    {
-        const int c4v = c >> 2;
-        float acc[16];
-#pragma unroll
-        for (int j = 0; j < 16; ++j) {
-            acc[j] = 0.f;
-            if (SMALL && j >= MJ) continue;
-            const int m = wave + 4 * j;
-#pragma unroll
-            for (int k = 0; k < 2; ++k) {
-                const int c4 = lane + 64 * k;
-                if (m < mid && c4 < c4v) {
-                    f32x4 wv;
-                    if constexpr (SMALL) wv = w1v[j < MJ ? j : 0][k];
-                    else wv = *(const f32x4*)(w1 + (long long)m * c + c4 * 4);
-                    const f32x4 pv = *(const f32x4*)(pooled + c4 * 4);
-                    acc[j] += wv.x * pv.x + wv.y * pv.y + wv.z * pv.z + wv.w * pv.w;
-                }
-            }
-        }
-#pragma unroll
-        for (int j = 0; j < 16; ++j) {
-            if (wave + 4 * j < mid) {
-                const float v = wave_sum(acc[j]);
-                if (lane == 0) hid[wave + 4 * j] = fmaxf(v, 0.f);
-            }
-        }
-    }
-    __syncthreads();
-    if constexpr (SMALL) {
-#pragma unroll
-        for (int q = 0; q < 2; ++q) {
-            const int ch = tid + 256 * q;
-            if (ch < c) {
-                float acc = 0.f;
-#pragma unroll
-                for (int m = 0; m < MW2; ++m)
-                    if (m < mid) acc += w2v[q][m] * hid[m];
-                gate[ch] = 1.0f / (1.0f + expf(-acc));
-            }
-        }
-    } else {
-        for (int ch = tid; ch < c; ch += 256) {
-            float acc = 0.f;
-#pragma unroll 8
-            for (int m = 0; m < mid; ++m) acc += w2[m * c + ch] * hid[m];
-            gate[ch] = 1.0f / (1.0f + expf(-acc));
-        }
-    }
-    __syncthreads();
+    const int img = blockIdx.y, tid = threadIdx.x;
+    se_gate<SMALL>(stats, tiles, c, mid, hw, w1, w2, img, pooled, hid, gate);
     const int c4n = c >> 2;
-    const long long base = ((long long)img * hw + (long long)blockIdx.x * rows) * c;
+    const long long pix0 = (long long)img * hw + (long long)blockIdx.x * rows;
+    const long long base = pix0 * c;
     const int total4 = rows * c4n;
     unsigned vm = 0u;
-    for (int i = tid; i < total4; i += 256) {
-        const int cc = i % c4n;
-        const f32x4 yy = *(const f32x4*)(y + base + (long long)i * 4);
-        const f32x4 rr = *(const f32x4*)(sc + base + (long long)i * 4);
-        const f32x4 ss = *(const f32x4*)&gate[cc * 4];
+    auto finish = [&](const f32x4 ss, const f32x4 yy, const f32x4 rr, long long off, long long pk) {
         f32x4 o = ss * yy + rr;
         if (packed) vm = range_acc(range_acc(range_acc(range_acc(vm, o.x), o.y), o.z), o.w);
         o.x = fmaxf(o.x, 0.f); o.y = fmaxf(o.y, 0.f); o.z = fmaxf(o.z, 0.f); o.w = fmaxf(o.w, 0.f);
-        if (out) *(f32x4*)(out + base + (long long)i * 4) = o;
-        if (packed) {
-            typedef _Float16 h4 __attribute__((ext_vector_type(4)));
-            const h4 hi = {(_Float16)o.x, (_Float16)o.y, (_Float16)o.z, (_Float16)o.w};
-            const h4 lo = {(_Float16)((o.x - (float)hi.x) * 2048.0f), (_Float16)((o.y - (float)hi.y) * 2048.0f),
-                           (_Float16)((o.z - (float)hi.z) * 2048.0f), (_Float16)((o.w - (float)hi.w) * 2048.0f)};
-            const long long pix = (long long)img * hw + (long long)blockIdx.x * rows + i / c4n;
-            *(h4*)(packed + pix * 2 * c + cc * 4) = hi;
-            *(h4*)(packed + pix * 2 * c + c + cc * 4) = lo;
+        if (out) *(f32x4*)(out + off) = o;
+        if (packed) store_pair(packed + pk, c, o);
+    };
+    if (256 % c4n == 0) {
+        const int cc = tid % c4n;
+        const f32x4 ss = *(const f32x4*)&gate[cc * 4];
+        long long off = base + (long long)tid * 4;
+        long long pk = (pix0 + tid / c4n) * 2 * c + cc * 4;
+        const long long ps = (long long)(256 / c4n) * 2 * c;
+        int i = tid;
+        for (; i + 3 * 256 < total4; i += 4 * 256) {
+            f32x4 yy[4], rr[4];
+#pragma unroll
+            for (int u = 0; u < 4; ++u) {
+                yy[u] = *(const f32x4*)(y + off + u * 1024);
+                rr[u] = *(const f32x4*)(sc + off + u * 1024);
+            }
+#pragma unroll
+            for (int u = 0; u < 4; ++u) finish(ss, yy[u], rr[u], off + u * 1024, pk + u * ps);
+            off += 4096;
+            pk += 4 * ps;
+        }
+        for (; i < total4; i += 256) {
+            finish(ss, *(const f32x4*)(y + off), *(const f32x4*)(sc + off), off, pk);
+            off += 1024;
+            pk += ps;
+        }
+    } else {
+        for (int i = tid; i < total4; i += 256) {
+            const int cc = i % c4n;
+            const long long off = base + (long long)i * 4;
+            finish(*(const f32x4*)&gate[cc * 4], *(const f32x4*)(y + off), *(const f32x4*)(sc + off), off,
+                   (pix0 + i / c4n) * 2 * c + cc * 4);
         }
     }
     range_raise(fault, vm);
 }
 
-__global__ __launch_bounds__(256) void gem_neck_kernel(const float* __restrict__ x, int hw, int c,
+__global__ __launch_bounds__(256, 4) void gem_neck_kernel(const float* __restrict__ x, int hw, int c,
                                                        const float* __restrict__ p_ptr, const float* __restrict__ scale,
                                                        const float* __restrict__ shift, float* __restrict__ gem_out,
-                                                       float* __restrict__ emb, int* __restrict__ fault) {
+                                                       float* __restrict__ emb, int* __restrict__ fault,
+                                                       const float* __restrict__ y, const float* __restrict__ sc,
+                                                       const float* __restrict__ stats, int tiles, int mid,
+                                                       const float* __restrict__ w1, const float* __restrict__ w2) {
     __shared__ float part[16][64 + 1];
-    const int img = blockIdx.y, c0 = blockIdx.x * 64;
+    __shared__ __attribute__((aligned(16))) float pooled[512];
+    __shared__ float hid[64];
+    __shared__ __attribute__((aligned(16))) float gate[512];
+    const int img = blockIdx.y;
     const int quad = threadIdx.x & 15, pg = threadIdx.x >> 4;
     const float p = p_ptr[0];
     const bool cube = p == 3.0f;
-    float acc[4] = {0.f, 0.f, 0.f, 0.f};
-    const float* xi = x + (long long)img * hw * c + c0 + quad * 4;
+    const bool tail = y != nullptr;
+    if (tail) se_gate<false>(stats, tiles, c, mid, hw, w1, w2, img, pooled, hid, gate);
     auto powp = [&](float f) {
         const float e = p * __builtin_amdgcn_logf(f);
         return e < -126.f ? __builtin_amdgcn_exp2f(e + 64.f) * 0x1p-64f : __builtin_amdgcn_exp2f(e);
     };
-    int px = pg;
-    for (; px + 7 * 16 < hw; px += 8 * 16) {
-        f32x4 v[8];
-#pragma unroll
-        for (int u = 0; u < 8; ++u) v[u] = *(const f32x4*)(xi + (long long)(px + 16 * u) * c);
-#pragma unroll
-        for (int u = 0; u < 8; ++u)
+    auto relu_fma = [](const f32x4 g, const f32x4 a, const f32x4 r) {
+        f32x4 o;
+#pragma unroll
+        for (int e = 0; e < 4; ++e) o[e] = fmaxf(__builtin_fmaf(g[e], a[e], r[e]), 0.f);
+        return o;
+    };
+    for (int c0 = blockIdx.x * 64; c0 < c; c0 += gridDim.x * 64) {
+        float acc[4] = {0.f, 0.f, 0.f, 0.f};
+        const long long ioff = (long long)img * hw * c + c0 + quad * 4;
+        const float* xi = (tail ? y : x) + ioff;
+        const float* si = tail ? sc + ioff : nullptr;
+        f32x4 gt = {0.f, 0.f, 0.f, 0.f};
+        if (tail) gt = *(const f32x4*)&gate[c0 + quad * 4];
+        auto add = [&](const f32x4 v) {
 #pragma unroll
             for (int e = 0; e < 4; ++e) {
-                const float f = fmaxf(v[u][e], 1e-6f);
+                const float f = fmaxf(v[e], 1e-6f);
                 acc[e] += cube ? f * f * f : powp(f);
             }
-    }
-    for (; px < hw; px += 16) {
-        const f32x4 v = *(const f32x4*)(xi + (long long)px * c);
-#pragma unroll
-        for (int e = 0; e < 4; ++e) {
-            const float f = fmaxf(v[e], 1e-6f);
-            acc[e] += cube ? f * f * f : powp(f);
-        }
-    }
-#pragma unroll
-    for (int e = 0; e < 4; ++e) part[pg][quad * 4 + e] = acc[e];
-    __syncthreads();
-    if (threadIdx.x < 64) {
-        float t = 0.f;
-#pragma unroll
-        for (int g = 0; g < 16; ++g) t += part[g][threadIdx.x];
-        const int ch = c0 + threadIdx.x;
-        const float m = t / (float)hw;
-        const float g = cube ? cbrtf(m) : powf(m, 1.0f / p);
-        if (gem_out) gem_out[(long long)img * c + ch] = g;
-        const float ev = g * scale[ch] + shift[ch];
-        emb[(long long)img * c + ch] = ev;
-        if (fault && !(fabsf(ev) < INFINITY)) fault[1] = 1;
+        };
+        int px = pg;
+        if (tail) {
+            for (; px + 3 * 16 < hw; px += 4 * 16) {
+                f32x4 v[4], r[4];
+#pragma unroll
+                for (int u = 0; u < 4; ++u) v[u] = *(const f32x4*)(xi + (long long)(px + 16 * u) * c);
+#pragma unroll
+                for (int u = 0; u < 4; ++u) r[u] = *(const f32x4*)(si + (long long)(px + 16 * u) * c);
+#pragma unroll
+                for (int u = 0; u < 4; ++u) add(relu_fma(gt, v[u], r[u]));
+            }
+        } else {
+            for (; px + 7 * 16 < hw; px += 8 * 16) {
+                f32x4 v[8];
+#pragma unroll
+                for (int u = 0; u < 8; ++u) v[u] = *(const f32x4*)(xi + (long long)(px + 16 * u) * c);
+#pragma unroll
+                for (int u = 0; u < 8; ++u) add(v[u]);
+            }
+        }
+        for (; px < hw; px += 16) {
+            f32x4 v = *(const f32x4*)(xi + (long long)px * c);
+            if (tail) v = relu_fma(gt, v, *(const f32x4*)(si + (long long)px * c));
+            add(v);
+        }
+#pragma unroll
+        for (int e = 0; e < 4; ++e) part[pg][quad * 4 + e] = acc[e];
+        __syncthreads();
+        if (threadIdx.x < 64) {
+            float t = 0.f;
+#pragma unroll
+            for (int g = 0; g < 16; ++g) t += part[g][threadIdx.x];
+            const int ch = c0 + threadIdx.x;
+            const float m = t / (float)hw;
+            const float g = cube ? cbrtf(m) : powf(m, 1.0f / p);
+            if (gem_out) gem_out[(long long)img * c + ch] = g;
+            const float ev = g * scale[ch] + shift[ch];
+            emb[(long long)img * c + ch] = ev;
+            if (fault && !(fabsf(ev) < INFINITY)) fault[1] = 1;
+        }
+        __syncthreads();
     }
 }
 
@@ -552,7 +675,21 @@
     ARG_CHECK(c % 64 == 0);
     prof_begin(ctx, REID_K_ELEMENTWISE, 0, (double)n_img * hw * c * 4.0);
     hipLaunchKernelGGL(gem_neck_kernel, dim3(c / 64, n_img), dim3(256), 0, ctx->stream, x, hw, c, p, scale, shift, gem_out, emb,
-                       ctx->fault);
+                       ctx->fault, nullptr, nullptr, nullptr, 0, 0, nullptr, nullptr);
+    prof_end(ctx);
+    LAUNCH_CHECK();
+    return REID_OK;
+}
+
+int launch_gem_neck_tail(reid_ctx* ctx, const float* stats, int n_img, int tiles, int c, int mid, int hw, const float* w1, const float* w2,
+                         const float* y, const float* sc, const float* p, const float* scale, const float* shift, float* gem_out,
+                         float* emb) {
+    ARG_CHECK(c % 64 == 0 && c <= 512 && mid <= 64 && y && sc && stats && w1 && w2);
+    int gx = 1;
+    while (gx < c / 64 && (long long)n_img * gx < 1024 && (c / 64) % (gx * 2) == 0) gx *= 2;
+    prof_begin(ctx, REID_K_ELEMENTWISE, 0, (double)n_img * hw * c * 8.0);
+    hipLaunchKernelGGL(gem_neck_kernel, dim3(gx, n_img), dim3(256), 0, ctx->stream, nullptr, hw, c, p, scale, shift, gem_out, emb,
+                       ctx->fault, y, sc, stats, tiles, mid, w1, w2);
     prof_end(ctx);
     LAUNCH_CHECK();
     return REID_OK;
diff --git a/real-time-reid-tracking_amd/csrc/reid_internal.h b/real-time-reid-tracking_amd/csrc/reid_internal.h
--- a/real-time-reid-tracking_amd/csrc/reid_internal.h
+++ b/real-time-reid-tracking_amd/csrc/reid_internal.h
@@ -264,6 +264,9 @@
                          bool in_half_only = false);
 int launch_gem_neck(reid_ctx*, const float* x, int n_img, int hw, int c, const float* p, const float* scale,
                     const float* shift, float* gem_out, float* emb);
+int launch_gem_neck_tail(reid_ctx*, const float* stats, int n_img, int tiles, int c, int mid, int hw, const float* w1, const float* w2,
+                         const float* y, const float* sc, const float* p, const float* scale, const float* shift, float* gem_out,
+                         float* emb);
 int launch_row_sqnorm(reid_ctx*, const float* x, int m, int d, long long ld, float* out);
 int launch_argmin_rows(reid_ctx*, const float* dist, int m, int n, long long ld, int32_t* idx, float* val);
 int launch_topk_rows(reid_ctx*, const float* dist, int m, int n, long long ld, int k, float* D, int32_t* I);
@@ -346,6 +349,7 @@
     int f16_loader_prio = 1;
     int f16_loader_waves = 1;
     int f16_halo = 1;
+    int gem_tail_min = 120;
     int f16_se_tail = 1;
     int f16_c64 = 2;
     int f16_stem_fused = 2;
diff --git a/real-time-reid-tracking_amd/engine.py b/real-time-reid-tracking_amd/engine.py
--- a/real-time-reid-tracking_amd/engine.py
+++ b/real-time-reid-tracking_amd/engine.py
@@ -509,6 +509,16 @@
             _ptr(_f32(shift)), _ptr(g), _ptr(e)))
         return g, e
 
+    def debug_gem_neck_fused(self, stats, w1, w2t, y, shortcut, p, scale, shift):
+        stats = _f32(stats)
+        n, tiles, c, _ = stats.shape
+        y, shortcut = _f32(y), _f32(shortcut)
+        g, e = np.empty((n, c), np.float32), np.empty((n, c), np.float32)
+        check(_ffi.debug_lib().reid_debug_gem_neck_fused(
+            self.h, C.c_int(n), C.c_int(y.shape[1]), C.c_int(c), C.c_int(w1.shape[0]), C.c_int(tiles), C.c_float(p), _ptr(stats),
+            _ptr(_f32(w1)), _ptr(_f32(w2t)), _ptr(y), _ptr(shortcut), _ptr(_f32(scale)), _ptr(_f32(shift)), _ptr(g), _ptr(e)))
+        return g, e
+
     def debug_stem(self, form, x, w, scale, shift):
         is_u8 = np.asarray(x).dtype == np.uint8
         x = np.ascontiguousarray(x, np.uint8) if is_u8 else _f32(x)
```

New measurement: 85660 crops/s (median of 6 runs). 1.9% higher.
